# sergivalverde/sub-cortical_segmentation

Hardware: NVIDIA B200
Metric: voxels_per_sec_full_volume_inference (higher is better)
Workload: dtype bf16

## Files before the change

sub-cortical_segmentation_b200/csrc/common.cuh:

```cuda
#pragma once
#include <cuda_bf16.h>
#include <cuda_runtime.h>
#include <nvtx3/nvToolsExt.h>
#include <stdint.h>
#include <stdio.h>
#include <atomic>
#include <string>
#include <utility>
#include <vector>

#include "../../include/subcort_b200.h"

namespace sc {

void set_error(const char* fmt, ...);

#define SC_CUDA(expr)                                                                        \
  do {                                                                                       \
    cudaError_t _e = (expr);                                                                 \
    if (_e != cudaSuccess) {                                                                 \
      sc::set_error("%s:%d: %s -> %s", __FILE__, __LINE__, #expr, cudaGetErrorString(_e));   \
      return SC_ERR_CUDA;                                                                    \
    }                                                                                        \
  } while (0)

#define SC_CHECK(cond, code, ...)   \
  do {                              \
    if (!(cond)) {                  \
      sc::set_error(__VA_ARGS__);   \
      return code;                  \
    }                               \
  } while (0)

#define SC_TRY(expr)           \
  do {                         \
    int _s = (expr);           \
    if (_s != SC_OK) return _s;\
  } while (0)

constexpr int kConvCin[5] = {1, 20, 20, 40, 40};
constexpr int kConvCout[5] = {20, 20, 40, 40, 60};

struct BranchOff {
  int convW[5];
  int bn[5][4];
  int alpha[5];
  int d1W, d1b, d1alpha;
};
struct ParamOff {
  BranchOff br[3];
  int fc1W, fc1b, a1;
  int fc2W, fc2b, a2;
  int outW, outb;
  int total;
};
inline ParamOff make_param_off() {
  ParamOff P;
  int o = 0;
  for (int b = 0; b < 3; ++b) {
    for (int l = 0; l < 5; ++l) {
      P.br[b].convW[l] = o; o += kConvCout[l] * kConvCin[l] * 9;
      for (int k = 0; k < 4; ++k) { P.br[b].bn[l][k] = o; o += kConvCout[l]; }
      P.br[b].alpha[l] = o; o += kConvCout[l];
    }
    P.br[b].d1W = o; o += 540 * 180;
    P.br[b].d1b = o; o += 180;
    P.br[b].d1alpha = o; o += 180;
  }
  P.fc1W = o; o += 540 * 540; P.fc1b = o; o += 540; P.a1 = o; o += 540;
  P.fc2W = o; o += 555 * 270; P.fc2b = o; o += 270; P.a2 = o; o += 270;
  P.outW = o; o += 270 * 15; P.outb = o; o += 15;
  P.total = o;
  return P;
}

constexpr int kFeat = 540;
constexpr int kFeatLd = 576;
constexpr int kH1 = 555;
constexpr int kH1Ld = 576;
constexpr int kH2 = 270;
constexpr int kH2Ld = 272;
constexpr int kH2LdTc = 320;
constexpr int kC5Ld = 64;
constexpr int kD1K = 9 * kC5Ld;

struct GemmW {
  float* w_kn;
  float* w_nk;
  float* bias;
  float* alpha;
  float* scale;
  int K, N, Kpad, Npad;
  int k_used = 0;
};

struct SweepW {
  float* panels;
  float* panels_pair;
  float* scale;
  float* shift;
  float* alpha;
  int bn, ksteps, npanels;
};

struct Conv1Consts { float w[9 * 20]; float scale[20], shift[20], alpha[20]; };

struct BranchW {
  Conv1Consts c1_host;
  float* c1_w;
  float* conv_w[5];
  float* scale[5];
  float* shift[5];
  float* alpha[5];
  SweepW conv_sw[5];
  GemmW d1;
  GemmW d1_dense;
};

struct Workspace {
  void* ptr = nullptr;
  size_t bytes = 0;
};

enum ProfClass {
  PC_GATHER = 0, PC_NONZERO, PC_SCATTER, PC_PATCH_BRANCH, PC_CONV1, PC_CONV2, PC_CONV3, PC_CONV4, PC_CONV5,
  PC_GEMM_D1, PC_GEMM_FC1, PC_GEMM_FC2, PC_ATLAS, PC_OUT, PC_POOL, PC_TRAIN_FWD, PC_TRAIN_BWD, PC_ADAM, PC_COUNT
};
struct ProfEvent { int cls; cudaEvent_t a, b; };

}

struct sc_ctx {
  int device = 0;
  int sm_count = 0;
  bool weights_loaded = false;
  int gemm_backend = 1;
  int64_t chunk_voxels = 1 << 20;
  int64_t launches = 0;
  sc::ParamOff off;
  float* params = nullptr;
  float* grads = nullptr;
  float* adam_m = nullptr;
  float* adam_v = nullptr;
  uint8_t* trainable = nullptr;
  int64_t adam_t = 0;
  float* derived = nullptr;
  size_t derived_floats = 0;
  sc::BranchW br[3];
  sc::GemmW fc1, fc2;
  sc::GemmW outl;
  float* out_w = nullptr;
  float* out_b = nullptr;
  sc::Workspace ws;
  sc::Workspace ws_train;
  sc::Workspace ws_fit;
  struct TrainGraph { int n; long long n_global; int injected; int backend; void* arena; cudaGraphExec_t exec; int launches; };
  std::vector<TrainGraph> train_graphs;
  cudaStream_t train_side[2] = {nullptr, nullptr};
  cudaEvent_t train_ev[8] = {};
  int train_graph_on = 1;
  unsigned* peer_flags = nullptr;
  float* peer_grads[8] = {}; float* peer_params[8] = {}; unsigned* peer_flagp[8] = {};
  int peer_rank = 0, peer_world = 0; unsigned peer_step = 0;
  sc_allreduce_fn ar_hook = nullptr;
  void* ar_user = nullptr;
  void* train_panels = nullptr;
  void* train_dense_w = nullptr;
  struct TrainDenseW { float* wnk; float* wkn; float* bias; };
  TrainDenseW train_dw[6];
  sc::SweepW train_sw[3][5][2];
  float* train_consts = nullptr;
  int64_t* d_count = nullptr;
  int64_t* h_count = nullptr;
  void* tc_state = nullptr;
  int tc_timing_cls = -1;
  unsigned long long* tc_timing_buf = nullptr;
  int train_wgrad_mn = 1;
  int train_fused_stats = 1;
  int tc_skip = 1;
  int tc_compact = 1;
  int32_t* h_slab_cnt = nullptr;
  unsigned char* tile_flags = nullptr;
  size_t tile_flags_cap = 0;
  cudaEvent_t compact_ev = nullptr;
  int gather_ctas_per_sm = 0;
  cudaStream_t copy_stream = nullptr;
  cudaEvent_t copy_ev[2] = {nullptr, nullptr};
  cudaEvent_t atlas_ready = nullptr;
  cudaEvent_t atlas_chunk_ev[64] = {};
  int atlas_chunks = 0, atlas_chunk_nx = 0;
  std::atomic<int>* atlas_recorded = nullptr;
  bool profile = false;
  std::vector<sc::ProfEvent> prof_live;
  std::vector<sc::ProfEvent> prof_free;
  bool derived_dirty = false;
  std::vector<std::pair<const void*, int>> smem_attr;
};

namespace sc {
int ensure_ws(Workspace& ws, size_t bytes);
int ensure_smem_attr(sc_ctx* ctx, const void* kernel, int bytes);

const char* prof_class_name(int cls);
struct ProfScope {
  sc_ctx* ctx; cudaStream_t st; ProfEvent ev; bool on;
  ProfScope(sc_ctx* c, int cls, cudaStream_t s) : ctx(c), st(s), on(c->profile) {
    nvtxRangePushA(prof_class_name(cls));
    if (!on) return;
    if (!ctx->prof_free.empty()) { ev = ctx->prof_free.back(); ctx->prof_free.pop_back(); }
    else { cudaEventCreate(&ev.a); cudaEventCreate(&ev.b); }
    ev.cls = cls;
    cudaEventRecord(ev.a, st);
  }
  ~ProfScope() {
    if (on) {
      cudaEventRecord(ev.b, st);
      ctx->prof_live.push_back(ev);
    }
    nvtxRangePop();
  }
};

struct OutGeo { int x0, y0, z0, by, bz, Y, Z; };

int launch_gather(sc_ctx* ctx, const float* vol, const int32_t* dims, const float* atlas, int bg_fix,
                  const int32_t* xyz, int64_t n, float* ax, float* co, float* sa, float* atlas_out, cudaStream_t st);
int launch_slab_compact(sc_ctx* ctx, const uint8_t* cand, const OutGeo& box, int bx, int nx_per_slab, int32_t* rowmap, int32_t* rowvox,
                        int32_t* cnt, int32_t* scratch, cudaStream_t st);
int launch_center_labels(sc_ctx* ctx, const uint8_t* lab, const int32_t* dims, const int32_t* xyz, int64_t n,
                         uint8_t* y, cudaStream_t st);
int launch_gather_samples(sc_ctx* ctx, const sc_scan* scans, int n_scans, const int32_t* samples, const float* atlas_rows,
                          const uint8_t* labels, const int64_t* idx, int64_t n, float* ax, float* co, float* sa,
                          float* atlas_out, uint8_t* y_out, cudaStream_t st);
int launch_nonzero(sc_ctx* ctx, const void* vol, int elem_bytes, const int32_t* dims, int32_t* xyz,
                   int64_t capacity, int64_t* n_out_host, cudaStream_t st);
int launch_dilate(sc_ctx* ctx, const uint8_t* mask, const int32_t* dims, int iterations, uint8_t* out, cudaStream_t st);
int launch_scatter(sc_ctx* ctx, const int32_t* xyz, int64_t n, const int32_t* label, const float* proba,
                   const int32_t* dims, uint8_t* label_vol, float* proba_vol, cudaStream_t st);

int import_volume(sc_ctx* ctx, const void* src, int elem_bytes, const int32_t* dims, int channels, void* dst, cudaStream_t st);
int upload_volume_box(sc_ctx* ctx, const void* src_host, int elem_bytes, const int32_t* dims, int channels, int fortran_order,
                      const int32_t* box, void* staging_dev, void* dst, cudaStream_t st);
int normalise_volume(sc_ctx* ctx, const void* vol, int dtype, const int32_t* dims, float* out, double* mean_std_host, cudaStream_t st);
int candidate_mask(sc_ctx* ctx, const void* vol, int dtype, const int32_t* dims, uint8_t* mask, cudaStream_t st);
int mask_bbox(sc_ctx* ctx, const uint8_t* mask, const int32_t* dims, int32_t* box_host, int64_t* count_host, cudaStream_t st);

int post_process(sc_ctx* ctx, const uint8_t* seg, const uint8_t* mask, const int32_t* dims, uint8_t* out, cudaStream_t st);

int derive_weights(sc_ctx* ctx, cudaStream_t st);

struct GemmProblem {
  const float* A;
  int64_t lda, a_ys, a_zs;
  int ntaps;
  int64_t tap_off[9];
  int kc;
  float* C;
  int64_t ldc, c_ys, c_zs;
  int M, Y, Z;
  const float* a_base;
  int64_t a_dims[4];
  int64_t a_strides[3];
  int tap_dx[9], tap_dy[9];
  int tap_dz[9] = {0, 0, 0, 0, 0, 0, 0, 0, 0};
  int a_y0, a_z0;
  int prof_cls;
  int k_used;
  int n_store;
  int c_col0;
  int out_split;
  const int32_t* rowmap = nullptr;
  const int32_t* rowvox = nullptr;
  const float* atlas = nullptr;
  OutGeo ageo;
  const struct SoftmaxOut* sm = nullptr;
  int a_swap = 0;
};
int launch_gemm(sc_ctx* ctx, const GemmProblem& p, const GemmW& w, cudaStream_t st);
inline void gemm_problem_rows(GemmProblem& p, const float* A, int64_t lda, int kc, int M) {
  p.c_col0 = 0; p.out_split = 0; p.k_used = 0; p.a_swap = 0;
  p.A = A; p.lda = lda; p.a_ys = p.a_zs = 0; p.ntaps = 1; p.tap_off[0] = 0; p.kc = kc;
  p.M = M; p.Y = p.Z = 1; p.c_ys = p.c_zs = 0;
  p.a_base = A; p.a_dims[0] = kc; p.a_dims[1] = M; p.a_dims[2] = p.a_dims[3] = 1;
  p.a_strides[0] = lda; p.a_strides[1] = p.a_strides[2] = (int64_t)M * lda;
  for (int t = 0; t < 9; ++t) p.tap_dx[t] = p.tap_dy[t] = 0;
  p.a_y0 = p.a_z0 = 0;
}
struct SoftmaxOut { float* proba; int32_t* label32; uint8_t* label8; const uint8_t* mask; OutGeo geo; int use_geo;
                    const int32_t* rowvox; };
int launch_out_softmax(sc_ctx* ctx, const float* h2, int64_t n, float* proba, int32_t* label32, uint8_t* label8,
                       const uint8_t* mask, const OutGeo* geo, cudaStream_t st);

int tc_init(sc_ctx* ctx);
void tc_destroy(sc_ctx* ctx);
int launch_gemm_tc(sc_ctx* ctx, const GemmProblem& p, const GemmW& w, cudaStream_t st);
int launch_split_rows(sc_ctx* ctx, const float* in, int64_t rows, float* out, cudaStream_t st);

struct ViewGeo {
  int64_t ss, rs, cs;
  int s0, ns;
  int r0, c0;
  int br, bc;
  int R, C;
};

int launch_conv1_wide(sc_ctx* ctx, const float* vol, const ViewGeo& g, int ns, const Conv1Consts& cw, float* out, int outR, int outC,
                      cudaStream_t st);
struct SweepStats { double* sums; int H, pitch; };
struct SweepSkip { const uint32_t* occ; int br, bc, ns, C1; uint8_t* flags; };
int launch_view_occupancy(sc_ctx* ctx, const uint8_t* cand, const ViewGeo& g, uint32_t* occ, cudaStream_t st);
int launch_conv_sweep(sc_ctx* ctx, const SweepW& w, int layer, const float* in, int in_fmt, float* out, int out_fmt,
                      int Pw, int R, int rows_out, int dil, int pool, int prof_cls, cudaStream_t st, int in_dx = 0, int in_dy = 0,
                      const SweepSkip* skip = nullptr, const struct SweepStats* stats = nullptr);

int launch_branch_patches(sc_ctx* ctx, int branch, const float* patches, int64_t n, float* c5_out ,
                          cudaStream_t st);
int forward_patches(sc_ctx* ctx, const float* in1, const float* in2, const float* in3, const float* in4, int64_t n,
                    float* proba, int32_t* label, cudaStream_t st);

struct ConvArgs {
  const float* in; int inR, inLd;
  float* out; int outR, outC, outLd;
  const float* w;
  const float* scale; const float* shift; const float* alpha;
  int ns; int round_out;
};
int launch_conv3x3(sc_ctx* ctx, int cin, int cout, const ConvArgs& a, int prof_cls, cudaStream_t st);
int launch_conv1_patches(sc_ctx* ctx, const float* patches, int n, const float* w, const float* scale, const float* shift,
                         const float* alpha, float* out, cudaStream_t st);
size_t branch_patches_tc_bytes(int64_t n);
int branch_patches_tc(sc_ctx* ctx, int branch, const float* patches, int64_t n, float* scratch, float* feats ,
                      cudaStream_t st);
int segment_volume(sc_ctx* ctx, const float* vol, const int32_t* dims, const float* atlas, const int32_t* box,
                   const uint8_t* cand, uint8_t* label_vol, float* proba_vol, cudaStream_t st);

constexpr float kBnEps = 1e-4f;
struct TcBranchBuf {
  float* X[5]; float* A[5]; uint16_t* AT[5]; uint8_t* idx[5]; float* mean[5]; float* istd[5];
  float* frame; float* dA; uint16_t* DT; float* dX0; double* sums;
};
size_t tc_branch_bytes(int n);
int tc_carve_branch(TcBranchBuf& T, char* base, int n);
int tc_branch_forward(sc_ctx* ctx, int b, const TcBranchBuf& T, const float* patches, const float* wf0, int n, const uint8_t* masks,
                      float* F5, cudaStream_t s);
int tc_branch_backward(sc_ctx* ctx, int b, const TcBranchBuf& T, const float* patches, const float* dF5, int dF5_ld, const uint8_t* masks, int n,
                       cudaStream_t s);
constexpr int kTrainZeros = 1024;
struct TcDenseBuf {
  int npad;
  char* zero_begin; size_t zero_bytes;
  float *F5s[3], *F5T[3], *Z1[3], *dZ1s[3], *dZ1T[3], *dF5[3], *gW1[3];
  float *CATs, *CATT, *ZF1, *CAT2s, *CAT2T, *ZF2, *H2s, *H2T, *ZO, *dZOs, *dZOT, *dH2, *dZF2s, *dZF2T, *dCAT2, *dZF1s, *dZF1T, *dCAT;
  float *gWfc1, *gWfc2, *gWout;
};
int tc_train_prepare(sc_ctx* ctx);
int tdense_prepare(sc_ctx* ctx);
size_t tdense_bytes(int n);
void tdense_carve(TcDenseBuf& D, char* base, int n);
int tdense_branch_forward(sc_ctx* ctx, int b, const TcDenseBuf& D, const float* F5, int n, const uint8_t* masks, cudaStream_t s);
int tdense_head(sc_ctx* ctx, const TcDenseBuf& D, const float* in4, const uint8_t* y, int n, int64_t n_global, const uint8_t* masks, float* loss,
                cudaStream_t s);
int tdense_branch_backward(sc_ctx* ctx, int b, const TcDenseBuf& D, int n, const uint8_t* masks, cudaStream_t s);
int launch_conv1_wgrad(sc_ctx* ctx, const float* patches, const float* dx_planar, int n, int zc, float* gW, cudaStream_t st);

int fused_export(sc_ctx* ctx, unsigned char* handles);
int fused_attach(sc_ctx* ctx, int rank, int world, const unsigned char* all);
void fused_detach(sc_ctx* ctx);
int fused_allreduce_adam(sc_ctx* ctx, float lr, float b1, float b2, float eps, cudaStream_t st);

int train_forward_backward(sc_ctx* ctx, const float* in1, const float* in2, const float* in3, const float* in4,
                           const uint8_t* y, int64_t n, int64_t n_global, uint64_t seed, const uint8_t* masks,
                           float* loss, cudaStream_t st);
int adam_step(sc_ctx* ctx, float lr, float b1, float b2, float eps, float gscale, float sscale, cudaStream_t st);
int eval_batch(sc_ctx* ctx, const float* in1, const float* in2, const float* in3, const float* in4, const uint8_t* y,
               int64_t n, float* out2, cudaStream_t st);

__device__ __forceinline__ float prelu(float x, float a) { return x > 0.f ? x : a * x; }
__device__ __forceinline__ void store_split4(float* row, int n, float v0, float v1, float v2, float v3) {
  __nv_bfloat16* r = reinterpret_cast<__nv_bfloat16*>(row) + (n >> 6) * 128 + (n & 63);
  const __nv_bfloat16 h0 = __float2bfloat16_rn(v0), h1 = __float2bfloat16_rn(v1), h2 = __float2bfloat16_rn(v2), h3 = __float2bfloat16_rn(v3);
  const __nv_bfloat16 l0 = __float2bfloat16_rn(v0 - __bfloat162float(h0)), l1 = __float2bfloat16_rn(v1 - __bfloat162float(h1));
  const __nv_bfloat16 l2 = __float2bfloat16_rn(v2 - __bfloat162float(h2)), l3 = __float2bfloat16_rn(v3 - __bfloat162float(h3));
  uint2 hp, lp;
  hp.x = (uint32_t)__bfloat16_as_ushort(h0) | ((uint32_t)__bfloat16_as_ushort(h1) << 16);
  hp.y = (uint32_t)__bfloat16_as_ushort(h2) | ((uint32_t)__bfloat16_as_ushort(h3) << 16);
  lp.x = (uint32_t)__bfloat16_as_ushort(l0) | ((uint32_t)__bfloat16_as_ushort(l1) << 16);
  lp.y = (uint32_t)__bfloat16_as_ushort(l2) | ((uint32_t)__bfloat16_as_ushort(l3) << 16);
  *reinterpret_cast<uint2*>(r) = hp;
  *reinterpret_cast<uint2*>(r + 64) = lp;
}
__device__ __forceinline__ void store_split4_b32(void* px, int n, float v0, float v1, float v2, float v3) {
  __nv_bfloat16* r = reinterpret_cast<__nv_bfloat16*>(px) + n;
  const __nv_bfloat16 h0 = __float2bfloat16_rn(v0), h1 = __float2bfloat16_rn(v1), h2 = __float2bfloat16_rn(v2), h3 = __float2bfloat16_rn(v3);
  const __nv_bfloat16 l0 = __float2bfloat16_rn(v0 - __bfloat162float(h0)), l1 = __float2bfloat16_rn(v1 - __bfloat162float(h1));
  const __nv_bfloat16 l2 = __float2bfloat16_rn(v2 - __bfloat162float(h2)), l3 = __float2bfloat16_rn(v3 - __bfloat162float(h3));
  uint2 hp, lp;
  hp.x = (uint32_t)__bfloat16_as_ushort(h0) | ((uint32_t)__bfloat16_as_ushort(h1) << 16);
  hp.y = (uint32_t)__bfloat16_as_ushort(h2) | ((uint32_t)__bfloat16_as_ushort(h3) << 16);
  lp.x = (uint32_t)__bfloat16_as_ushort(l0) | ((uint32_t)__bfloat16_as_ushort(l1) << 16);
  lp.y = (uint32_t)__bfloat16_as_ushort(l2) | ((uint32_t)__bfloat16_as_ushort(l3) << 16);
  *reinterpret_cast<uint2*>(r) = hp;
  *reinterpret_cast<uint2*>(r + 32) = lp;
}
__device__ __forceinline__ void store_row1(float* row, int n, int split, float v) {
  if (!split) { row[n] = v; return; }
  __nv_bfloat16* r = reinterpret_cast<__nv_bfloat16*>(row) + (n >> 6) * 128 + (n & 63);
  const __nv_bfloat16 h = __float2bfloat16_rn(v);
  r[0] = h;
  r[64] = __float2bfloat16_rn(v - __bfloat162float(h));
}
__device__ __forceinline__ void store_row4(float* row, int n, int split, float v0, float v1, float v2, float v3) {
  if (split) store_split4(row, n, v0, v1, v2, v3);
  else *reinterpret_cast<float4*>(row + n) = make_float4(v0, v1, v2, v3);
}
}
```

sub-cortical_segmentation_b200/csrc/dense.cu:

```cuda
#include <thread>

#include "common.cuh"

namespace sc {


__host__ __device__ inline int round8(int v) { return (v + 7) & ~7; }

__global__ void __launch_bounds__(256) dense_conv1_kernel(const float* __restrict__ vol, ViewGeo g, int sbeg, int ns,
                                                          const float* __restrict__ w, const float* __restrict__ scale,
                                                          const float* __restrict__ shift, const float* __restrict__ alpha,
                                                          float* __restrict__ out, int outR, int ld) {
  __shared__ float sw[9 * 20], ssc[20], ssh[20], sal[20];
  for (int i = threadIdx.x; i < 180; i += 256) sw[i] = w[i];
  if (threadIdx.x < 20) { ssc[threadIdx.x] = scale[threadIdx.x]; ssh[threadIdx.x] = shift[threadIdx.x]; sal[threadIdx.x] = alpha[threadIdx.x]; }
  __syncthreads();
  const int quads = ld >> 2;
  const int64_t total = (int64_t)ns * outR * quads;
  for (int64_t e = (int64_t)blockIdx.x * 256 + threadIdx.x; e < total; e += (int64_t)gridDim.x * 256) {
    const int q = (int)(e % quads);
    const int i = (int)((e / quads) % outR);
    const int s = (int)(e / ((int64_t)quads * outR));
    const int j0 = q * 4;
    float x[3][6];
    const float* base = vol + (int64_t)(g.s0 + sbeg + s) * g.ss;
#pragma unroll
    for (int ky = 0; ky < 3; ++ky) {
      const int rr = g.r0 + i + ky - 16;
      const bool rin = rr >= 0 && rr < g.R;
#pragma unroll
      for (int t = 0; t < 6; ++t) {
        const int cc = g.c0 + j0 + t - 16;
        x[ky][t] = (rin && cc >= 0 && cc < g.C) ? __ldg(base + (int64_t)rr * g.rs + (int64_t)cc * g.cs) : 0.f;
      }
    }
    float* o = out + (((int64_t)s * 20) * outR + i) * ld + j0;
    const int64_t plane = (int64_t)outR * ld;
#pragma unroll 4
    for (int co = 0; co < 20; ++co) {
      float a0 = 0.f, a1 = 0.f, a2 = 0.f, a3 = 0.f;
#pragma unroll
      for (int ky = 0; ky < 3; ++ky)
#pragma unroll
        for (int kx = 0; kx < 3; ++kx) {
          const float wv = sw[(ky * 3 + kx) * 20 + co];
          a0 = fmaf(x[ky][kx + 0], wv, a0); a1 = fmaf(x[ky][kx + 1], wv, a1);
          a2 = fmaf(x[ky][kx + 2], wv, a2); a3 = fmaf(x[ky][kx + 3], wv, a3);
        }
      const float sc_ = ssc[co], sh = ssh[co], al = sal[co];
      float4 v;
      v.x = prelu(fmaf(a0, sc_, sh), al); v.y = prelu(fmaf(a1, sc_, sh), al);
      v.z = prelu(fmaf(a2, sc_, sh), al); v.w = prelu(fmaf(a3, sc_, sh), al);
      *reinterpret_cast<float4*>(o + co * plane) = v;
    }
  }
}

template <int CIN, int COUT, int DIL, int POOLD, bool NHWC_OUT>
struct ConvCfg {
  static constexpr int TH = 16, TW = 32, CHUNK = 10;
  static constexpr int CO_T = COUT / 5;
  static constexpr int IH = TH + 2 * DIL;
  static constexpr int NV = (8 + 2 * DIL + 3) / 4;
  static constexpr int IW = 24 + NV * 4;
  static constexpr int IWP = (IW % 8 == 4) ? IW : IW + 4;
  static constexpr int IN_FLOATS = CHUNK * IH * IWP;
  static constexpr int W_FLOATS = CHUNK * 9 * COUT;
  static constexpr size_t SMEM = (size_t)(IN_FLOATS + W_FLOATS) * sizeof(float);
};

template <int CIN, int COUT, int DIL, int POOLD, bool NHWC_OUT>
__global__ void __launch_bounds__(320) dense_conv_kernel(const ConvArgs a) {
  using Cfg = ConvCfg<CIN, COUT, DIL, POOLD, NHWC_OUT>;
  extern __shared__ __align__(16) float smem[];
  float* s_in = smem;
  float* s_w = smem + Cfg::IN_FLOATS;
  const int tid = threadIdx.x;
  const int cg = tid >> 6, pg = tid & 63, prow = pg >> 2, pseg = pg & 3;
  const int tr0 = blockIdx.y * Cfg::TH, tc0 = blockIdx.x * Cfg::TW;
  const int s = blockIdx.z;
  const float* in_s = a.in + (int64_t)s * CIN * a.inR * a.inLd;

  float acc[8][Cfg::CO_T];
#pragma unroll
  for (int p = 0; p < 8; ++p)
#pragma unroll
    for (int c = 0; c < Cfg::CO_T; ++c) acc[p][c] = 0.f;

  for (int ci0 = 0; ci0 < CIN; ci0 += Cfg::CHUNK) {
    __syncthreads();
    for (int e = tid; e < Cfg::CHUNK * Cfg::IH * Cfg::IW; e += 320) {
      const int col = e % Cfg::IW;
      const int row = (e / Cfg::IW) % Cfg::IH;
      const int ci = e / (Cfg::IW * Cfg::IH);
      const int gr = tr0 + row, gc = tc0 + col;
      float v = 0.f;
      if (gr + POOLD < a.inR && gc + POOLD < a.inLd) {
        const float* p = in_s + ((int64_t)(ci0 + ci) * a.inR + gr) * a.inLd + gc;
        v = __ldg(p);
        if (POOLD > 0) {
          v = fmaxf(v, __ldg(p + POOLD));
          v = fmaxf(v, fmaxf(__ldg(p + (int64_t)POOLD * a.inLd), __ldg(p + (int64_t)POOLD * a.inLd + POOLD)));
        }
      }
      s_in[(ci * Cfg::IH + row) * Cfg::IWP + col] = v;
    }
    for (int e = tid; e < Cfg::W_FLOATS / 4; e += 320)
      reinterpret_cast<float4*>(s_w)[e] = __ldg(reinterpret_cast<const float4*>(a.w + (int64_t)ci0 * 9 * COUT) + e);
    __syncthreads();

#pragma unroll 1
    for (int ci = 0; ci < Cfg::CHUNK; ++ci) {
#pragma unroll
      for (int ky = 0; ky < 3; ++ky) {
        float x[Cfg::NV * 4];
        const float4* src = reinterpret_cast<const float4*>(s_in + (ci * Cfg::IH + prow + ky * DIL) * Cfg::IWP + pseg * 8);
#pragma unroll
        for (int v = 0; v < Cfg::NV; ++v) {
          const float4 t = src[v];
          x[v * 4 + 0] = t.x; x[v * 4 + 1] = t.y; x[v * 4 + 2] = t.z; x[v * 4 + 3] = t.w;
        }
#pragma unroll
        for (int kx = 0; kx < 3; ++kx) {
          float wv[Cfg::CO_T];
          const float4* wsrc = reinterpret_cast<const float4*>(s_w + (ci * 9 + ky * 3 + kx) * COUT + cg * Cfg::CO_T);
#pragma unroll
          for (int v = 0; v < Cfg::CO_T / 4; ++v) {
            const float4 t = wsrc[v];
            wv[v * 4 + 0] = t.x; wv[v * 4 + 1] = t.y; wv[v * 4 + 2] = t.z; wv[v * 4 + 3] = t.w;
          }
#pragma unroll
          for (int p = 0; p < 8; ++p)
#pragma unroll
            for (int c = 0; c < Cfg::CO_T; ++c) acc[p][c] = fmaf(x[kx * DIL + p], wv[c], acc[p][c]);
        }
      }
    }
  }

  const int orow = tr0 + prow, ocol = tc0 + pseg * 8;
  if (orow >= a.outR) return;
  if (!NHWC_OUT) {
    if (ocol >= a.outLd) return;
#pragma unroll
    for (int c = 0; c < Cfg::CO_T; ++c) {
      const int co = cg * Cfg::CO_T + c;
      const float sc_ = __ldg(a.scale + co), sh = __ldg(a.shift + co), al = __ldg(a.alpha + co);
      float r[8];
#pragma unroll
      for (int p = 0; p < 8; ++p) r[p] = prelu(fmaf(acc[p][c], sc_, sh), al);
      float* o = a.out + (((int64_t)s * COUT + co) * a.outR + orow) * a.outLd + ocol;
      *reinterpret_cast<float4*>(o) = make_float4(r[0], r[1], r[2], r[3]);
      *reinterpret_cast<float4*>(o + 4) = make_float4(r[4], r[5], r[6], r[7]);
    }
  } else {
    float sc_[Cfg::CO_T], sh[Cfg::CO_T], al[Cfg::CO_T];
#pragma unroll
    for (int c = 0; c < Cfg::CO_T; ++c) {
      const int co = cg * Cfg::CO_T + c;
      sc_[c] = __ldg(a.scale + co); sh[c] = __ldg(a.shift + co); al[c] = __ldg(a.alpha + co);
    }
#pragma unroll
    for (int p = 0; p < 8; ++p) {
      if (ocol + p >= a.outC) break;
      float* o = a.out + (((int64_t)s * a.outR + orow) * a.outC + ocol + p) * kC5Ld;
#pragma unroll
      for (int v = 0; v < Cfg::CO_T / 4; ++v) {
        float r[4];
#pragma unroll
        for (int k = 0; k < 4; ++k) r[k] = prelu(fmaf(acc[p][v * 4 + k], sc_[v * 4 + k], sh[v * 4 + k]), al[v * 4 + k]);
        store_row4(o, cg * Cfg::CO_T + v * 4, a.round_out, r[0], r[1], r[2], r[3]);
      }
      if (cg == 4 && COUT < kC5Ld) store_row4(o, COUT, a.round_out, 0.f, 0.f, 0.f, 0.f);
    }
  }
}

template <int CIN, int COUT, int DIL, int POOLD, bool NHWC_OUT>
static int launch_dense_conv(sc_ctx* ctx, const ConvArgs& a, int prof_cls, cudaStream_t st) {
  using Cfg = ConvCfg<CIN, COUT, DIL, POOLD, NHWC_OUT>;
  auto kern = dense_conv_kernel<CIN, COUT, DIL, POOLD, NHWC_OUT>;
  SC_TRY(ensure_smem_attr(ctx, reinterpret_cast<const void*>(kern), (int)Cfg::SMEM));
  const int width = NHWC_OUT ? a.outC : a.outLd;
  dim3 grid((width + Cfg::TW - 1) / Cfg::TW, (a.outR + Cfg::TH - 1) / Cfg::TH, a.ns);
  ProfScope prof(ctx, prof_cls, st);
  kern<<<grid, 320, Cfg::SMEM, st>>>(a);
  ctx->launches++;
  SC_CUDA(cudaGetLastError());
  return SC_OK;
}

size_t branch_patches_tc_bytes(int64_t n) {
  return (size_t)n * ((960 + 240) * 32 + (240 + 56 + 56) * 64) * sizeof(float) + 5 * 256;
}

int branch_patches_tc(sc_ctx* ctx, int b, const float* patches, int64_t n, float* scratch, float* feats, cudaStream_t st) {
  const BranchW& W = ctx->br[b];
  auto carve = [&](float*& cur, size_t floats) { float* p = cur; cur += (floats + 63) & ~(size_t)63; return p; };
  float* cur = scratch;
  float* c1 = carve(cur, (size_t)n * 960 * 32);
  float* p1 = carve(cur, (size_t)n * 240 * 32);
  float* c3 = carve(cur, (size_t)n * 240 * 64);
  float* p2 = carve(cur, (size_t)n * 56 * 64);
  float* c5 = carve(cur, (size_t)n * 56 * 64);
  SC_CHECK(n * 960 < (1ll << 31), SC_ERR_ARG, "patchwise chunk too large");
  {
    ViewGeo g = {1024, 32, 1, 0, (int)n, 16, 16, 30, 30, 32, 32};
    SC_TRY(launch_conv1_wide(ctx, patches, g, (int)n, W.c1_host, c1, 30, 32, st));
  }
  SC_TRY(launch_conv_sweep(ctx, W.conv_sw[1], 1, c1, 1, p1, 1, (int)(n * 32), 30, 28, 1, 2, PC_CONV2, st));
  SC_TRY(launch_conv_sweep(ctx, W.conv_sw[2], 2, p1, 1, c3, 0, (int)(n * 16), 15, 12, 1, 0, PC_CONV3, st));
  SC_TRY(launch_conv_sweep(ctx, W.conv_sw[3], 3, c3, 0, p2, 0, (int)(n * 16), 15, 10, 1, 2, PC_CONV4, st));
  SC_TRY(launch_conv_sweep(ctx, W.conv_sw[4], 4, p2, 0, c5, 0, (int)(n * 8), 7, 3, 1, 0, PC_CONV5, st));
  GemmProblem p;
  p.A = c5; p.lda = 8 * kC5Ld; p.a_ys = 0; p.a_zs = 0;
  p.ntaps = 9; p.kc = kC5Ld; p.k_used = 0;
  for (int t = 0; t < 9; ++t) {
    p.tap_dx[t] = 0; p.tap_dy[t] = t % 3; p.tap_dz[t] = t / 3;
    p.tap_off[t] = ((int64_t)(t / 3) * n * 8 + (t % 3)) * kC5Ld;
  }
  p.a_base = c5; p.a_dims[0] = kC5Ld; p.a_dims[1] = n; p.a_dims[2] = 8; p.a_dims[3] = 7;
  p.a_strides[0] = 8 * kC5Ld; p.a_strides[1] = kC5Ld; p.a_strides[2] = (int64_t)n * 8 * kC5Ld;
  p.a_y0 = p.a_z0 = 0;
  p.C = feats; p.ldc = kFeatLd; p.c_ys = p.c_zs = 0; p.M = (int)n; p.Y = p.Z = 1;
  p.n_store = 192; p.c_col0 = b * 192; p.out_split = 1; p.prof_cls = PC_GEMM_D1;
  SC_TRY(launch_gemm_tc(ctx, p, W.d1_dense, st));
  SC_CUDA(cudaGetLastError());
  return SC_OK;
}

int launch_conv3x3(sc_ctx* ctx, int cin, int cout, const ConvArgs& a, int prof_cls, cudaStream_t st) {
  if (cin == 20 && cout == 20) return launch_dense_conv<20, 20, 1, 0, false>(ctx, a, prof_cls, st);
  if (cin == 20 && cout == 40) return launch_dense_conv<20, 40, 1, 0, false>(ctx, a, prof_cls, st);
  if (cin == 40 && cout == 40) return launch_dense_conv<40, 40, 1, 0, false>(ctx, a, prof_cls, st);
  if (cin == 40 && cout == 60) return launch_dense_conv<40, 60, 1, 0, false>(ctx, a, prof_cls, st);
  if (cin == 60 && cout == 40) return launch_dense_conv<60, 40, 1, 0, false>(ctx, a, prof_cls, st);
  if (cin == 40 && cout == 20) return launch_dense_conv<40, 20, 1, 0, false>(ctx, a, prof_cls, st);
  set_error("launch_conv3x3: unsupported channel pair %d -> %d", cin, cout);
  return SC_ERR_ARG;
}

int launch_conv1_patches(sc_ctx* ctx, const float* patches, int n, const float* w, const float* scale, const float* shift,
                         const float* alpha, float* out, cudaStream_t st) {
  ViewGeo g = {1024, 32, 1, 0, n, 16, 16, 30, 30, 32, 32};
  const int64_t work = (int64_t)n * 30 * 8;
  const int64_t blocks = (work + 255) / 256;
  const unsigned grid = (unsigned)(blocks < (int64_t)ctx->sm_count * 32 ? blocks : (int64_t)ctx->sm_count * 32);
  ProfScope prof(ctx, PC_TRAIN_FWD, st);
  dense_conv1_kernel<<<grid, 256, 0, st>>>(patches, g, 0, n, w, scale, shift, alpha, out, 30, 32);
  ctx->launches++;
  SC_CUDA(cudaGetLastError());
  return SC_OK;
}

__global__ void dense_atlas_kernel(const float* __restrict__ atlas, OutGeo g, int ix0, int64_t rows, float* __restrict__ h1,
                                   int split) {
  const int64_t m = (int64_t)blockIdx.x * blockDim.x + threadIdx.x;
  if (m >= rows) return;
  const int64_t plane = (int64_t)g.by * g.bz;
  const int ix = (int)(m / plane);
  const int rem = (int)(m - (int64_t)ix * plane);
  const int iy = rem / g.bz, iz = rem - iy * g.bz;
  const int64_t v = ((int64_t)(g.x0 + ix0 + ix) * g.Y + (g.y0 + iy)) * g.Z + (g.z0 + iz);
  float a[16];
#pragma unroll
  for (int c = 0; c < 15; ++c) a[c] = __ldg(atlas + v * 15 + c);
  float s = __fadd_rn(__fadd_rn(__fadd_rn(a[0], a[1]), __fadd_rn(a[2], a[3])),
                      __fadd_rn(__fadd_rn(a[4], a[5]), __fadd_rn(a[6], a[7])));
#pragma unroll
  for (int k = 8; k < 15; ++k) s = __fadd_rn(s, a[k]);
  if (s == 0.f) a[14] = 1.f;
  a[15] = 0.f;
  float* hr = h1 + m * kH1Ld;
#pragma unroll
  for (int q = 0; q < 9; ++q) {
    if (q < 4) store_row4(hr, 540 + 4 * q, split, a[4 * q], a[4 * q + 1], a[4 * q + 2], a[4 * q + 3]);
    else store_row4(hr, 540 + 4 * q, split, 0.f, 0.f, 0.f, 0.f);
  }
}

static size_t align256(size_t v) { return (v + 255) & ~(size_t)255; }

int segment_volume(sc_ctx* ctx, const float* vol, const int32_t* dims, const float* atlas, const int32_t* box,
                   const uint8_t* cand, uint8_t* label_vol, float* proba_vol, cudaStream_t st) {
  const int X = dims[0], Y = dims[1], Z = dims[2];
  int b[6] = {0, X, 0, Y, 0, Z};
  if (box) for (int i = 0; i < 6; ++i) b[i] = box[i];
  SC_CHECK(b[0] >= 0 && b[1] <= X && b[2] >= 0 && b[3] <= Y && b[4] >= 0 && b[5] <= Z, SC_ERR_ARG, "sc_segment_volume: box outside the volume");
  const int bx = b[1] - b[0], by = b[3] - b[2], bz = b[5] - b[4];
  if (bx <= 0 || by <= 0 || bz <= 0) return SC_OK;
  const int64_t YZ = (int64_t)Y * Z;
  const bool tc = ctx->gemm_backend == 1;

  ViewGeo vg[3];
  vg[0] = {1, YZ, Z, b[4], bz, b[0], b[2], bx, by, X, Y};
  vg[1] = {Z, YZ, 1, b[2], by, b[0], b[4], bx, bz, X, Z};
  vg[2] = {YZ, Z, 1, b[0], bx, b[2], b[4], by, bz, Y, Z};

  size_t a5_off[3], a5_bytes = 0;
  for (int v = 0; v < 3; ++v) {
    a5_off[v] = a5_bytes;
    a5_bytes += tc ? align256((size_t)vg[v].ns * (vg[v].br + 29) * (vg[v].bc + 29) * kC5Ld * sizeof(float))
                   : align256((size_t)vg[v].ns * (vg[v].br + 8) * (vg[v].bc + 8) * kC5Ld * sizeof(float));
  }
  size_t per_slice_max = 0, view_max = 0;
  for (int v = 0; v < 3; ++v) {
    const size_t br = vg[v].br, bc = vg[v].bc;
    size_t f;
    if (tc) {
      f = (size_t)vg[v].ns * (br + 29) * (bc + 29) * (2 * 32 + 2 * 64) + 4 * 64;
      view_max = f > view_max ? f : view_max;
      continue;
    }
    f = 20 * (br + 29) * round8(bc + 29) + 20 * (br + 27) * round8(bc + 27) + 40 * (br + 22) * round8(bc + 22) +
        40 * (br + 18) * round8(bc + 18);
    per_slice_max = f > per_slice_max ? f : per_slice_max;
  }
  const size_t scratch_budget = (size_t)1536 << 20;
  int group = tc ? 1 : (int)(scratch_budget / (per_slice_max * sizeof(float) + 1024));
  if (group < 1) group = 1;
  if (group > 64) group = 64;
  const size_t scratch_bytes = tc ? align256(view_max * sizeof(float) + 4096) : align256((per_slice_max * sizeof(float) + 1024) * group);
  const int64_t plane = (int64_t)by * bz;
  int slab = (int)(ctx->chunk_voxels / plane);
  if (slab < 1) slab = 1;
  if (slab > bx) slab = bx;
  const size_t rows_max = (size_t)slab * plane;
  const size_t feat_bytes = align256(rows_max * kFeatLd * sizeof(float));
  const size_t h1_bytes = align256(rows_max * kH1Ld * sizeof(float));
  const int h2ld = tc ? kH2LdTc : kH2Ld;
  const size_t h2_bytes = align256(rows_max * h2ld * sizeof(float));
  const int nslabs = (bx + slab - 1) / slab;
  bool compact = tc && cand != nullptr && ctx->tc_compact && nslabs <= 4096;
  const size_t nbox = (size_t)bx * plane;
  const size_t cmp_blocks = (size_t)nslabs * ((rows_max + 2047) / 2048);
  const size_t cmp_bytes = compact ? align256(nbox * 4) * 2 + align256(cmp_blocks * 8 + 16) + align256((size_t)nslabs * 4) : 0;
  size_t occ_off[3], skip_bytes = 0;
  for (int v = 0; v < 3; ++v) { occ_off[v] = skip_bytes; skip_bytes += compact ? align256((size_t)vg[v].br * vg[v].ns * 4) : 0; }
  const size_t flags_off = skip_bytes;
  if (compact) skip_bytes += align256((size_t)1 << 20);
  const size_t total = a5_bytes + scratch_bytes + feat_bytes + h1_bytes + h2_bytes + cmp_bytes + skip_bytes;
  SC_TRY(ensure_ws(ctx->ws, total));
  char* wsb = reinterpret_cast<char*>(ctx->ws.ptr);
  float* a5[3] = {reinterpret_cast<float*>(wsb + a5_off[0]), reinterpret_cast<float*>(wsb + a5_off[1]),
                  reinterpret_cast<float*>(wsb + a5_off[2])};
  char* scratch = wsb + a5_bytes;
  float* feats = reinterpret_cast<float*>(scratch + scratch_bytes);
  float* h1 = reinterpret_cast<float*>(reinterpret_cast<char*>(feats) + feat_bytes);
  float* h2 = reinterpret_cast<float*>(reinterpret_cast<char*>(h1) + h1_bytes);
  int32_t* rowmap = reinterpret_cast<int32_t*>(reinterpret_cast<char*>(h2) + h2_bytes);
  int32_t* rowvox = reinterpret_cast<int32_t*>(reinterpret_cast<char*>(rowmap) + align256(nbox * 4));
  int32_t* cmp_scratch = reinterpret_cast<int32_t*>(reinterpret_cast<char*>(rowvox) + align256(nbox * 4));
  int32_t* d_slab_cnt = reinterpret_cast<int32_t*>(reinterpret_cast<char*>(cmp_scratch) + align256(cmp_blocks * 8 + 16));
  char* skip_base = wsb + (total - skip_bytes);
  if (compact) {
    if (!ctx->h_slab_cnt) {
      SC_CUDA(cudaMallocHost(&ctx->h_slab_cnt, 4096 * sizeof(int32_t)));
      SC_CUDA(cudaEventCreateWithFlags(&ctx->compact_ev, cudaEventDisableTiming));
    }
    OutGeo boxg = {b[0], b[2], b[4], by, bz, Y, Z};
    SC_TRY(launch_slab_compact(ctx, cand, boxg, bx, slab, rowmap, rowvox, d_slab_cnt, cmp_scratch, st));
    SC_CUDA(cudaMemcpyAsync(ctx->h_slab_cnt, d_slab_cnt, (size_t)nslabs * sizeof(int32_t), cudaMemcpyDeviceToHost, st));
    SC_CUDA(cudaEventRecord(ctx->compact_ev, st));
    SC_CUDA(cudaEventSynchronize(ctx->compact_ev));
    int64_t ncand = 0;
    for (int i = 0; i < nslabs; ++i) ncand += ctx->h_slab_cnt[i];
    if (ncand * 10 >= (int64_t)nbox * 9) compact = false;
  }
  SweepSkip skips[3];
  const bool skip_on = compact && ctx->tc_skip;
  if (skip_on) {
    for (int v = 0; v < 3; ++v) {
      uint32_t* occ = reinterpret_cast<uint32_t*>(skip_base + occ_off[v]);
      SC_TRY(launch_view_occupancy(ctx, cand, vg[v], occ, st));
      skips[v] = {occ, vg[v].br, vg[v].bc, vg[v].ns, vg[v].bc + 29, reinterpret_cast<uint8_t*>(skip_base + flags_off)};
    }
  }

  for (int v = 0; v < 3; ++v) {
    const ViewGeo& g = vg[v];
    const BranchW& W = ctx->br[v];
    const int r1 = g.br + 29, l1 = round8(g.bc + 29);
    const int r2 = g.br + 27, l2 = round8(g.bc + 27);
    const int r3 = g.br + 22, l3 = round8(g.bc + 22);
    const int r4 = g.br + 18, l4 = round8(g.bc + 18);
    const int r5 = g.br + 8, c5 = g.bc + 8;
    if (tc) {
      const int R1 = g.br + 29, C1 = g.bc + 29;
      const int64_t Pw64 = (int64_t)g.ns * C1;
      const int64_t npos = Pw64 * R1;
      SC_CHECK(npos < (1ll << 31), SC_ERR_ARG, "sc_segment_volume: view too large");
      const int Pw = (int)Pw64;
      auto carve = [&](float*& cur, int px_floats) { float* p = cur; cur += align256((size_t)npos * px_floats * 4) / 4; return p; };
      float* cur = reinterpret_cast<float*>(scratch);
      float* m1 = carve(cur, 32); float* mp1 = carve(cur, 32);
      float* m3 = carve(cur, 64); float* mp2 = carve(cur, 64);
      SC_TRY(launch_conv1_wide(ctx, vol, g, g.ns, W.c1_host, m1, R1, C1, st));
      const SweepSkip* sk = skip_on ? &skips[v] : nullptr;
      SC_TRY(launch_conv_sweep(ctx, W.conv_sw[1], 1, m1, 1, mp1, 1, Pw, R1, g.br + 26, 1, 1, PC_CONV2, st, 0, 0, sk));
      SC_TRY(launch_conv_sweep(ctx, W.conv_sw[2], 2, mp1, 1, m3, 0, Pw, R1, g.br + 22, 2, 0, PC_CONV3, st, 0, 0, sk));
      SC_TRY(launch_conv_sweep(ctx, W.conv_sw[3], 3, m3, 0, mp2, 0, Pw, R1, g.br + 16, 2, 1, PC_CONV4, st, 0, 0, sk));
      SC_TRY(launch_conv_sweep(ctx, W.conv_sw[4], 4, mp2, 0, a5[v], 0, Pw, R1, g.br + 8, 4, 0, PC_CONV5, st, 0, 0, sk));
      SC_CUDA(cudaGetLastError());
    }
    for (int sb = 0; sb < g.ns && !tc; sb += group) {
      const int ns = g.ns - sb < group ? g.ns - sb : group;
      float* c1 = reinterpret_cast<float*>(scratch);
      float* c2 = c1 + align256((size_t)ns * 20 * r1 * l1 * 4) / 4;
      float* c3 = c2 + align256((size_t)ns * 20 * r2 * l2 * 4) / 4;
      float* c4 = c3 + align256((size_t)ns * 40 * r3 * l3 * 4) / 4;
      {
        const int64_t work = (int64_t)ns * r1 * (l1 / 4);
        const int64_t blocks = (work + 255) / 256;
        const unsigned grid = (unsigned)(blocks < (int64_t)ctx->sm_count * 32 ? blocks : (int64_t)ctx->sm_count * 32);
        ProfScope prof(ctx, PC_CONV1, st);
        dense_conv1_kernel<<<grid, 256, 0, st>>>(vol, g, sb, ns, W.c1_w, W.scale[0], W.shift[0], W.alpha[0], c1, r1, l1);
        ctx->launches++;
        SC_CUDA(cudaGetLastError());
      }
      ConvArgs a;
      a.ns = ns; a.round_out = 0;
      a.in = c1; a.inR = r1; a.inLd = l1; a.out = c2; a.outR = r2; a.outC = g.bc + 27; a.outLd = l2;
      a.w = W.conv_w[1]; a.scale = W.scale[1]; a.shift = W.shift[1]; a.alpha = W.alpha[1];
      SC_TRY((launch_dense_conv<20, 20, 1, 0, false>(ctx, a, PC_CONV2, st)));
      a.in = c2; a.inR = r2; a.inLd = l2; a.out = c3; a.outR = r3; a.outC = g.bc + 22; a.outLd = l3;
      a.w = W.conv_w[2]; a.scale = W.scale[2]; a.shift = W.shift[2]; a.alpha = W.alpha[2];
      SC_TRY((launch_dense_conv<20, 40, 2, 1, false>(ctx, a, PC_CONV3, st)));
      a.in = c3; a.inR = r3; a.inLd = l3; a.out = c4; a.outR = r4; a.outC = g.bc + 18; a.outLd = l4;
      a.w = W.conv_w[3]; a.scale = W.scale[3]; a.shift = W.shift[3]; a.alpha = W.alpha[3];
      SC_TRY((launch_dense_conv<40, 40, 2, 0, false>(ctx, a, PC_CONV4, st)));
      a.in = c4; a.inR = r4; a.inLd = l4; a.out = a5[v] + (size_t)sb * r5 * c5 * kC5Ld; a.outR = r5; a.outC = c5; a.outLd = c5;
      a.w = W.conv_w[4]; a.scale = W.scale[4]; a.shift = W.shift[4]; a.alpha = W.alpha[4];
      a.round_out = tc ? 1 : 0;
      SC_TRY((launch_dense_conv<40, 60, 4, 2, true>(ctx, a, PC_CONV5, st)));
    }
  }

  int atlas_waited = 0;
  OutGeo og = {b[0], b[2], b[4], by, bz, Y, Z};
  if (tc) SC_CUDA(cudaMemsetAsync(h2, 0, h2_bytes, st));
  for (int ix0 = 0; ix0 < bx; ix0 += slab) {
    const int nx = bx - ix0 < slab ? bx - ix0 : slab;
    const int64_t rows = (int64_t)nx * plane;
    if (ctx->atlas_chunks > 0) {
      int need = (b[0] + ix0 + nx + ctx->atlas_chunk_nx - 1) / ctx->atlas_chunk_nx;
      if (need > ctx->atlas_chunks) need = ctx->atlas_chunks;
      if (need > atlas_waited) {
        if (ctx->atlas_recorded)
          while (ctx->atlas_recorded->load(std::memory_order_acquire) < need) std::this_thread::yield();
        SC_CUDA(cudaStreamWaitEvent(st, ctx->atlas_chunk_ev[need - 1], 0));
        atlas_waited = need;
      }
    }
    const int64_t slab_base = (int64_t)ix0 * plane;
    const int64_t rows_fc = compact ? ctx->h_slab_cnt[ix0 / slab] : rows;
    if (rows_fc == 0) continue;
    for (int v = 0; v < 3; ++v) {
      const ViewGeo& g = vg[v];
      const int64_t c5 = tc ? g.bc + 29 : g.bc + 8, r5 = tc ? g.br + 29 : g.br + 8;
      GemmProblem p;
      p.lda = kC5Ld; p.a_ys = c5 * kC5Ld; p.a_zs = r5 * c5 * kC5Ld;
      p.ntaps = 9; p.kc = kC5Ld;
      for (int t = 0; t < 9; ++t) {
        p.tap_off[t] = ((int64_t)(t / 3) * 4 * c5 + (t % 3) * 4) * kC5Ld;
        p.tap_dx[t] = (t % 3) * 4; p.tap_dy[t] = (t / 3) * 4;
      }
      p.a_base = a5[v]; p.a_dims[0] = kC5Ld; p.a_dims[1] = c5; p.a_dims[2] = r5; p.a_dims[3] = g.ns;
      p.a_strides[0] = kC5Ld; p.a_strides[1] = c5 * kC5Ld; p.a_strides[2] = r5 * c5 * kC5Ld;
      p.a_swap = 0;
      if (tc) {
        p.a_dims[2] = g.ns; p.a_dims[3] = r5;
        p.a_strides[1] = c5 * kC5Ld; p.a_strides[2] = (int64_t)g.ns * c5 * kC5Ld;
        p.a_swap = 1;
      }
      p.a_y0 = v == 2 ? 0 : ix0; p.a_z0 = v == 2 ? ix0 : 0;
      p.ldc = 0; p.out_split = tc ? 1 : 0; p.c_col0 = v * 192; p.prof_cls = PC_GEMM_D1; p.k_used = 0;
      p.n_store = 192;
      if (v == 0) {
        p.A = a5[0] + (int64_t)ix0 * p.a_ys; p.M = by; p.Y = nx; p.Z = bz;
        p.ldc = (int64_t)bz * kFeatLd; p.c_ys = plane * kFeatLd; p.c_zs = kFeatLd;
      } else if (v == 1) {
        p.A = a5[1] + (int64_t)ix0 * p.a_ys; p.M = bz; p.Y = nx; p.Z = by;
        p.ldc = kFeatLd; p.c_ys = plane * kFeatLd; p.c_zs = (int64_t)bz * kFeatLd;
      } else {
        p.A = a5[2] + (int64_t)ix0 * p.a_zs; p.M = bz; p.Y = by; p.Z = nx;
        p.ldc = kFeatLd; p.c_ys = (int64_t)bz * kFeatLd; p.c_zs = plane * kFeatLd;
      }
      p.C = feats;
      if (compact) p.rowmap = rowmap + slab_base;
      SC_TRY(tc ? launch_gemm_tc(ctx, p, ctx->br[v].d1_dense, st) : launch_gemm(ctx, p, ctx->br[v].d1_dense, st));
    }
    GemmProblem p;
    SC_CHECK(rows < (1ll << 31), SC_ERR_ARG, "sc_segment_volume: chunk too large");
    gemm_problem_rows(p, feats, kFeatLd, kFeatLd, (int)rows_fc);
    p.C = h1; p.ldc = kH1Ld; p.n_store = 540; p.out_split = tc ? 1 : 0;
    p.prof_cls = PC_GEMM_FC1;
    const bool atlas_fused = tc;
    if (ctx->atlas_ready && ctx->atlas_chunks == 0) {
      SC_CUDA(cudaStreamWaitEvent(st, ctx->atlas_ready, 0));
      ctx->atlas_ready = nullptr;
    }
    if (atlas_fused) { p.atlas = atlas; p.ageo = og; p.ageo.x0 = b[0] + ix0; if (compact) p.rowvox = rowvox + slab_base; }
    SC_TRY(tc ? launch_gemm_tc(ctx, p, ctx->fc1, st) : launch_gemm(ctx, p, ctx->fc1, st));
    p.atlas = nullptr; p.rowvox = nullptr;
    if (!atlas_fused) {
      ProfScope prof(ctx, PC_ATLAS, st);
      dense_atlas_kernel<<<(unsigned)((rows + 255) / 256), 256, 0, st>>>(atlas, og, ix0, rows, h1, tc ? 1 : 0);
      ctx->launches++;
    }
    SC_CUDA(cudaGetLastError());
    gemm_problem_rows(p, h1, kH1Ld, kH1Ld, (int)rows_fc);
    p.C = h2; p.ldc = h2ld; p.n_store = kH2Ld; p.out_split = tc ? 1 : 0;
    p.prof_cls = PC_GEMM_FC2;
    SC_TRY(tc ? launch_gemm_tc(ctx, p, ctx->fc2, st) : launch_gemm(ctx, p, ctx->fc2, st));
    OutGeo og2 = og;
    og2.x0 = b[0] + ix0;
    if (tc) {
      SoftmaxOut smo = {proba_vol, nullptr, label_vol, cand, og2, 1, compact ? rowvox + slab_base : nullptr};
      gemm_problem_rows(p, h2, h2ld, h2ld, (int)rows_fc);
      p.C = nullptr; p.ldc = 0; p.n_store = 16; p.out_split = 0; p.sm = &smo;
      p.prof_cls = PC_OUT;
      SC_TRY(launch_gemm_tc(ctx, p, ctx->outl, st));
    } else {
      SC_TRY(launch_out_softmax(ctx, h2, rows, proba_vol, nullptr, label_vol, cand, &og2, st));
    }
  }
  if (ctx->atlas_ready && ctx->atlas_chunks == 0) {
    SC_CUDA(cudaStreamWaitEvent(st, ctx->atlas_ready, 0));
    ctx->atlas_ready = nullptr;
  }
  return SC_OK;
}

}
```

sub-cortical_segmentation_b200/csrc/gemm_simt.cu:

```cuda
#include "common.cuh"

namespace sc {

constexpr int BM = 128, BN = 64, BK = 16;
constexpr int AS_LD = BM + 4;

struct GemmArgs {
  GemmProblem p;
  const float* W;
  const float* bias;
  const float* alpha;
  int Npad;
  int mt, nt;
};

__global__ void __launch_bounds__(256) gemm_simt_kernel(const GemmArgs a) {
  __shared__ __align__(16) float As[BK][AS_LD];
  __shared__ __align__(16) float Bs[BK][BN];
  const GemmProblem& p = a.p;
  int64_t bid = blockIdx.x;
  const int n_tile = (int)(bid % a.nt); bid /= a.nt;
  const int m_tile = (int)(bid % a.mt); bid /= a.mt;
  const int y = (int)(bid % p.Y);
  const int z = (int)(bid / p.Y);
  const int m0 = m_tile * BM, n0 = n_tile * BN;
  const float* Abase = p.A + (int64_t)z * p.a_zs + (int64_t)y * p.a_ys;
  const int tid = threadIdx.x, tm = tid & 15, tn = tid >> 4;

  float acc[8][4];
#pragma unroll
  for (int i = 0; i < 8; ++i)
#pragma unroll
    for (int j = 0; j < 4; ++j) acc[i][j] = 0.f;

  for (int tap = 0; tap < p.ntaps; ++tap) {
    const float* At = Abase + p.tap_off[tap];
    const float* Wt = a.W + (int64_t)tap * p.kc * a.Npad;
    for (int k0 = 0; k0 < p.kc; k0 += BK) {
#pragma unroll
      for (int r = 0; r < 2; ++r) {
        const int idx = tid + r * 256, row = idx >> 2, kq = idx & 3;
        float4 v = make_float4(0.f, 0.f, 0.f, 0.f);
        if (m0 + row < p.M) v = __ldg(reinterpret_cast<const float4*>(At + (int64_t)(m0 + row) * p.lda + k0 + kq * 4));
        As[kq * 4 + 0][row] = v.x; As[kq * 4 + 1][row] = v.y; As[kq * 4 + 2][row] = v.z; As[kq * 4 + 3][row] = v.w;
      }
      {
        const int kr = tid >> 4, nq = tid & 15;
        float4 v = make_float4(0.f, 0.f, 0.f, 0.f);
        if (n0 + nq * 4 < a.Npad) v = __ldg(reinterpret_cast<const float4*>(Wt + (int64_t)(k0 + kr) * a.Npad + n0 + nq * 4));
        *reinterpret_cast<float4*>(&Bs[kr][nq * 4]) = v;
      }
      __syncthreads();
#pragma unroll
      for (int k = 0; k < BK; ++k) {
        const float4 a0 = *reinterpret_cast<const float4*>(&As[k][tm * 8]);
        const float4 a1 = *reinterpret_cast<const float4*>(&As[k][tm * 8 + 4]);
        const float4 b = *reinterpret_cast<const float4*>(&Bs[k][tn * 4]);
        const float av[8] = {a0.x, a0.y, a0.z, a0.w, a1.x, a1.y, a1.z, a1.w};
        const float bv[4] = {b.x, b.y, b.z, b.w};
#pragma unroll
        for (int i = 0; i < 8; ++i)
#pragma unroll
          for (int j = 0; j < 4; ++j) acc[i][j] = fmaf(av[i], bv[j], acc[i][j]);
      }
      __syncthreads();
    }
  }
  const int n = n0 + tn * 4;
  if (n >= p.n_store) return;
  const float4 bias = __ldg(reinterpret_cast<const float4*>(a.bias + n));
  const float4 al = __ldg(reinterpret_cast<const float4*>(a.alpha + n));
  float* Cbase = p.C + (int64_t)z * p.c_zs + (int64_t)y * p.c_ys;
#pragma unroll
  for (int i = 0; i < 8; ++i) {
    const int m = m0 + tm * 8 + i;
    if (m >= p.M) break;
    float4 v;
    v.x = prelu(acc[i][0] + bias.x, al.x);
    v.y = prelu(acc[i][1] + bias.y, al.y);
    v.z = prelu(acc[i][2] + bias.z, al.z);
    v.w = prelu(acc[i][3] + bias.w, al.w);
    *reinterpret_cast<float4*>(Cbase + (int64_t)m * p.ldc + p.c_col0 + n) = v;
  }
}

int launch_gemm(sc_ctx* ctx, const GemmProblem& p, const GemmW& w, cudaStream_t st) {
  if (p.M <= 0 || p.Y <= 0 || p.Z <= 0) return SC_OK;
  SC_CHECK(p.kc % BK == 0 && p.n_store % 4 == 0 && p.n_store <= w.Npad, SC_ERR_ARG, "gemm: bad geometry kc=%d n_store=%d", p.kc, p.n_store);
  SC_CHECK(p.ntaps * p.kc == w.Kpad, SC_ERR_ARG, "gemm: K mismatch %d*%d vs %d", p.ntaps, p.kc, w.Kpad);
  SC_CHECK(!p.out_split && p.c_col0 % 4 == 0, SC_ERR_ARG, "gemm: the SIMT back-end writes plain fp32 rows only");
  GemmArgs a;
  a.p = p; a.W = w.w_kn; a.bias = w.bias; a.alpha = w.alpha; a.Npad = w.Npad;
  a.mt = (p.M + BM - 1) / BM;
  a.nt = (p.n_store + BN - 1) / BN;
  const int64_t blocks = (int64_t)a.mt * a.nt * p.Y * p.Z;
  SC_CHECK(blocks < (1ll << 31), SC_ERR_ARG, "gemm: grid too large");
  ProfScope prof(ctx, p.prof_cls, st);
  gemm_simt_kernel<<<(unsigned)blocks, 256, 0, st>>>(a);
  ctx->launches++;
  SC_CUDA(cudaGetLastError());
  return SC_OK;
}

__global__ void __launch_bounds__(128) out_softmax_kernel(const float* __restrict__ h2, int64_t n,
                                                          const float* __restrict__ W, const float* __restrict__ b,
                                                          float* __restrict__ proba, int32_t* __restrict__ label,
                                                          uint8_t* __restrict__ label8, const uint8_t* __restrict__ mask,
                                                          const OutGeo geo, const int use_geo) {
  __shared__ __align__(16) float sW[270 * 16];
  for (int i = threadIdx.x; i < 270 * 16; i += 128) sW[i] = W[i];
  __syncthreads();
  const int64_t v = (int64_t)blockIdx.x * 128 + threadIdx.x;
  if (v >= n) return;
  int64_t o = v;
  if (use_geo) {
    const int64_t plane = (int64_t)geo.by * geo.bz;
    const int ix = (int)(v / plane);
    const int rem = (int)(v - (int64_t)ix * plane);
    const int iy = rem / geo.bz, iz = rem - iy * geo.bz;
    o = ((int64_t)(geo.x0 + ix) * geo.Y + (geo.y0 + iy)) * geo.Z + (geo.z0 + iz);
    if (mask && mask[o] == 0) return;
  }
  const float4* row = reinterpret_cast<const float4*>(h2 + v * kH2Ld);
  float z[15];
#pragma unroll
  for (int c = 0; c < 15; ++c) z[c] = __ldg(b + c);
#pragma unroll 2
  for (int k4 = 0; k4 < 68; ++k4) {
    const float4 xv = __ldg(row + k4);
    const float x[4] = {xv.x, xv.y, xv.z, xv.w};
#pragma unroll
    for (int j = 0; j < 4; ++j) {
      const int k = k4 * 4 + j;
      if (k < 270) {
        const float4* w4 = reinterpret_cast<const float4*>(sW + k * 16);
        const float4 w0 = w4[0], w1 = w4[1], w2 = w4[2], w3 = w4[3];
        z[0] = fmaf(x[j], w0.x, z[0]); z[1] = fmaf(x[j], w0.y, z[1]); z[2] = fmaf(x[j], w0.z, z[2]); z[3] = fmaf(x[j], w0.w, z[3]);
        z[4] = fmaf(x[j], w1.x, z[4]); z[5] = fmaf(x[j], w1.y, z[5]); z[6] = fmaf(x[j], w1.z, z[6]); z[7] = fmaf(x[j], w1.w, z[7]);
        z[8] = fmaf(x[j], w2.x, z[8]); z[9] = fmaf(x[j], w2.y, z[9]); z[10] = fmaf(x[j], w2.z, z[10]); z[11] = fmaf(x[j], w2.w, z[11]);
        z[12] = fmaf(x[j], w3.x, z[12]); z[13] = fmaf(x[j], w3.y, z[13]); z[14] = fmaf(x[j], w3.z, z[14]);
      }
    }
  }
  float mx = z[0];
#pragma unroll
  for (int c = 1; c < 15; ++c) mx = fmaxf(mx, z[c]);
  float sum = 0.f;
#pragma unroll
  for (int c = 0; c < 15; ++c) { z[c] = expf(z[c] - mx); sum += z[c]; }
  const float inv = 1.f / sum;
  int best = 0;
  float bp = z[0] * inv;
#pragma unroll
  for (int c = 0; c < 15; ++c) {
    z[c] *= inv;
    if (z[c] > bp) { bp = z[c]; best = c; }
  }
  if (proba) {
#pragma unroll
    for (int c = 0; c < 15; ++c) proba[o * 15 + c] = z[c];
  }
  if (label) label[o] = best;
  if (label8) label8[o] = (uint8_t)best;
}

int launch_out_softmax(sc_ctx* ctx, const float* h2, int64_t n, float* proba, int32_t* label, uint8_t* label8,
                       const uint8_t* mask, const OutGeo* geo, cudaStream_t st) {
  if (n == 0) return SC_OK;
  const int64_t blocks = (n + 127) / 128;
  SC_CHECK(blocks < (1ll << 31), SC_ERR_ARG, "out_softmax: too many rows");
  const unsigned grid = (unsigned)blocks;
  OutGeo g = geo ? *geo : OutGeo{0, 0, 0, 1, 1, 1, 1};
  ProfScope prof(ctx, PC_OUT, st);
  out_softmax_kernel<<<grid, 128, 0, st>>>(h2, n, ctx->out_w, ctx->out_b, proba, label, label8, mask, g, geo ? 1 : 0);
  ctx->launches++;
  SC_CUDA(cudaGetLastError());
  return SC_OK;
}

}
```

sub-cortical_segmentation_b200/csrc/gemm_tc.cu:

```cuda
#include "tc_common.cuh"

namespace sc {

__device__ __forceinline__ void tmem_ld16(uint32_t (&r)[16], uint32_t taddr) {
  asm volatile(
      "tcgen05.ld.sync.aligned.32x32b.x16.b32 {%0, %1, %2, %3, %4, %5, %6, %7, %8, %9, %10, %11, %12, %13, %14, %15}, [%16];"
      : "=r"(r[0]), "=r"(r[1]), "=r"(r[2]), "=r"(r[3]), "=r"(r[4]), "=r"(r[5]), "=r"(r[6]), "=r"(r[7]), "=r"(r[8]),
        "=r"(r[9]), "=r"(r[10]), "=r"(r[11]), "=r"(r[12]), "=r"(r[13]), "=r"(r[14]), "=r"(r[15])
      : "r"(taddr));
}

constexpr int TC_BM = 128;
constexpr int TC_BK = 64;
constexpr int TC_A_HALF = TC_BM * 128;

struct TcArgs {
  int kpt;
  int nkb;
  int stages;
  int bn;
  int nt, mt;
  int Y;
  int M;
  int n_store, npad, c_col0;
  int a_y0, a_z0;
  int a_swap;
  int tap_dx[9], tap_dy[9], tap_dz[9];
  float* C;
  long long ldc, c_ys, c_zs;
  const float* bias;
  const float* alpha;
  const float* scale;
  int out_split;
  long long num_tiles;
  int epi_warps;
  int last_ksteps;
  unsigned long long* dbg;
  const int* rowmap;
  const int* rowvox;
  long long crow_ld;
  int n_mma;
  const unsigned char* tile_on;
  const float* atlas;
  OutGeo ageo;
  int sm_on;
  SoftmaxOut sm;
};


__global__ void __launch_bounds__(576, 1)
gemm_tc_persistent_kernel(const __grid_constant__ CUtensorMap mapA, const __grid_constant__ CUtensorMap mapB, const TcArgs a) {
  extern __shared__ uint8_t smem_raw[];
  uint8_t* smem = smem_raw + ((1024u - (smem_u32(smem_raw) & 1023u)) & 1023u);
  const int b_half = a.bn * 128;
  const int w_block = 2 * b_half;
  const int stage_bytes = 2 * TC_A_HALF + w_block;
  uint8_t* sStage = smem;
  uint64_t* bars = reinterpret_cast<uint64_t*>(sStage + a.stages * stage_bytes);
  uint64_t* full = bars;
  uint64_t* empty = bars + a.stages;
  uint64_t* tfull = bars + 2 * a.stages;
  uint64_t* tempty = tfull + 2;
  uint32_t* tmem_slot = reinterpret_cast<uint32_t*>(tempty + 2);
  float* s_const = reinterpret_cast<float*>(tmem_slot + 4);
  uint8_t* s_stage = reinterpret_cast<uint8_t*>(s_const + 2 * 3 * a.bn);

  const int warp = threadIdx.x >> 5, lane = threadIdx.x & 31;

  if (threadIdx.x == 0) {
    for (int s = 0; s < a.stages; ++s) { mbar_init(&full[s], 1); mbar_init(&empty[s], 1); }
    for (int b = 0; b < 2; ++b) { mbar_init(&tfull[b], 1); mbar_init(&tempty[b], (blockDim.x >> 5) - 2); }
    asm volatile("fence.mbarrier_init.release.cluster;" ::: "memory");
  }
  if (warp == 1) {
    asm volatile("tcgen05.alloc.cta_group::1.sync.aligned.shared::cta.b32 [%0], %1;" ::"r"(smem_u32(tmem_slot)), "r"(512) : "memory");
    asm volatile("tcgen05.relinquish_alloc_permit.cta_group::1.sync.aligned;" ::: "memory");
  }
  asm volatile("tcgen05.fence::before_thread_sync;" ::: "memory");
  __syncthreads();
  asm volatile("tcgen05.fence::after_thread_sync;" ::: "memory");
  const uint32_t tmem_base = *tmem_slot;

  if (warp == 0) {
    if (lane == 0) {
      asm volatile("prefetch.tensormap [%0];" ::"l"(reinterpret_cast<uint64_t>(&mapA)) : "memory");
      asm volatile("prefetch.tensormap [%0];" ::"l"(reinterpret_cast<uint64_t>(&mapB)) : "memory");
      uint32_t it = 0;
      long long dbg_acc[1] = {0};
      const long long tstart = a.dbg ? clock64() : 0;
      for (long long t = blockIdx.x; t < a.num_tiles; t += gridDim.x) {
        long long r = t;
        const int n_tile = (int)(r % a.nt); r /= a.nt;
        const int m_tile = (int)(r % a.mt); r /= a.mt;
        const int y = (int)(r % a.Y);
        const int z = (int)(r / a.Y);
        const int m0 = m_tile * TC_BM, n0 = n_tile * a.bn;
        for (int kb = 0; kb < a.nkb; ++kb, ++it) {
          const int s = it % a.stages;
          const uint32_t use = it / a.stages;
          if (use > 0) {
            const long long c0 = a.dbg ? clock64() : 0;
            mbar_wait(&empty[s], (use - 1) & 1);
            if (a.dbg) dbg_acc[0] += clock64() - c0;
          }
          mbar_expect_tx(&full[s], (uint32_t)stage_bytes);
          uint8_t* sp = sStage + s * stage_bytes;
          const int tap = kb / a.kpt, ka = (kb - tap * a.kpt) * 2 * TC_BK;
          const int px = m0 + a.tap_dx[tap], ln = y + a.a_y0 + a.tap_dy[tap], pl = z + a.a_z0 + a.tap_dz[tap];
          tma_load_4d(&mapA, &full[s], sp, ka, px, a.a_swap ? pl : ln, a.a_swap ? ln : pl);
          tma_load_4d(&mapA, &full[s], sp + TC_A_HALF, ka + TC_BK, px, a.a_swap ? pl : ln, a.a_swap ? ln : pl);
          tma_load_2d(&mapB, &full[s], sp + 2 * TC_A_HALF, kb * 2 * TC_BK, n0);
          tma_load_2d(&mapB, &full[s], sp + 2 * TC_A_HALF + b_half, kb * 2 * TC_BK + TC_BK, n0);
        }
      }
      if (a.dbg) { a.dbg[blockIdx.x * 8 + 0] = (unsigned long long)dbg_acc[0]; a.dbg[blockIdx.x * 8 + 1] = (unsigned long long)(clock64() - tstart); }
    }
    __syncwarp();
  } else if (warp == 1) {
    const uint32_t leader = elect_one();
    const uint32_t idesc = (1u << 4) | (1u << 7) | (1u << 10) | ((uint32_t)(a.bn >> 3) << 17) | ((uint32_t)(TC_BM >> 4) << 24);
    const uint32_t sStage_u = smem_u32(sStage);
    uint32_t it = 0, ti = 0;
    long long w_full = 0, w_tempty = 0;
    const long long tstart = a.dbg ? clock64() : 0;
    for (long long t = blockIdx.x; t < a.num_tiles; t += gridDim.x, ++ti) {
      const uint32_t b = ti & 1, buse = ti >> 1;
      long long c0 = a.dbg ? clock64() : 0;
      mbar_wait(&tempty[b], (buse & 1) ^ 1);
      if (a.dbg) w_tempty += clock64() - c0;
      asm volatile("tcgen05.fence::after_thread_sync;" ::: "memory");
      const uint32_t acc = tmem_base + b * 256;
      for (int kb = 0; kb < a.nkb; ++kb, ++it) {
        const int s = it % a.stages;
        c0 = a.dbg ? clock64() : 0;
        mbar_wait(&full[s], (it / a.stages) & 1);
        if (a.dbg) w_full += clock64() - c0;
        asm volatile("tcgen05.fence::after_thread_sync;" ::: "memory");
        const uint32_t sp = sStage_u + s * stage_bytes;
        const uint64_t ah = umma_desc(sp), al = umma_desc(sp + TC_A_HALF);
        const uint64_t wh = umma_desc(sp + 2 * TC_A_HALF), wl = umma_desc(sp + 2 * TC_A_HALF + b_half);
#pragma unroll
        for (int j = 0; j < 4; ++j) {
          const uint64_t o = (uint64_t)(j * 2);
          umma_bf16_elect(acc, al + o, wh + o, idesc, (kb | j) != 0, leader);
          umma_bf16_elect(acc, ah + o, wl + o, idesc, 1, leader);
          umma_bf16_elect(acc, ah + o, wh + o, idesc, 1, leader);
        }
        if (leader) umma_commit(&empty[s]);
        __syncwarp();
      }
      if (leader) umma_commit(&tfull[b]);
      __syncwarp();
    }
    if (a.dbg && leader) {
      a.dbg[blockIdx.x * 8 + 2] = (unsigned long long)w_full; a.dbg[blockIdx.x * 8 + 3] = (unsigned long long)w_tempty;
      a.dbg[blockIdx.x * 8 + 4] = (unsigned long long)(clock64() - tstart);
    }
  } else {
    const int q = warp & 3;
    const int nepi = (blockDim.x >> 5) - 2, G = nepi >> 2, grp = (warp - 2) >> 2;
    const int epi_threads = nepi * 32;
    uint32_t ti = 0;
    long long w_tfull = 0;
    const long long tstart = a.dbg ? clock64() : 0;
    for (long long t = blockIdx.x; t < a.num_tiles; t += gridDim.x, ++ti) {
      long long r = t;
      const int n_tile = (int)(r % a.nt); r /= a.nt;
      const int m_tile = (int)(r % a.mt); r /= a.mt;
      const int y = (int)(r % a.Y);
      const int z = (int)(r / a.Y);
      const int m0 = m_tile * TC_BM, n0 = n_tile * a.bn;
      const uint32_t b = ti & 1, buse = ti >> 1;
      float* cb = s_const + b * 3 * a.bn;
      if (ti < 2 || a.nt > 1) {
        for (int i = threadIdx.x - 64; i < a.bn; i += epi_threads) {
          const int nn = n0 + i;
          const bool ok = nn < a.npad;
          cb[i] = ok ? __ldg(a.bias + nn) : 0.f;
          cb[a.bn + i] = ok ? __ldg(a.alpha + nn) : 1.f;
          cb[2 * a.bn + i] = (a.scale && ok) ? __ldg(a.scale + nn) : 1.f;
        }
        asm volatile("bar.sync 1, %0;" ::"r"(epi_threads) : "memory");
      }
      const long long c0w = a.dbg ? clock64() : 0;
      mbar_wait(&tfull[b], buse & 1);
      if (a.dbg) w_tfull += clock64() - c0w;
      asm volatile("tcgen05.fence::after_thread_sync;" ::: "memory");
      float* ctile = a.C + (long long)z * a.c_zs + (long long)y * a.c_ys;
      const int mw = m0 + q * 32;
      uint8_t* stg = s_stage + (warp - 2) * 2560;
      uint8_t* mine = stg + lane * 80;
      if (a.sm_on) {
        if (grp == 0) {
          uint32_t rr[16];
          const uint32_t taddr = tmem_base + b * 256 + ((uint32_t)(q * 32) << 16);
          asm volatile(
              "tcgen05.ld.sync.aligned.32x32b.x16.b32 {%0, %1, %2, %3, %4, %5, %6, %7, %8, %9, %10, %11, %12, %13, %14, %15}, [%16];"
              : "=r"(rr[0]), "=r"(rr[1]), "=r"(rr[2]), "=r"(rr[3]), "=r"(rr[4]), "=r"(rr[5]), "=r"(rr[6]), "=r"(rr[7]), "=r"(rr[8]),
                "=r"(rr[9]), "=r"(rr[10]), "=r"(rr[11]), "=r"(rr[12]), "=r"(rr[13]), "=r"(rr[14]), "=r"(rr[15])
              : "r"(taddr));
          asm volatile("tcgen05.wait::ld.sync.aligned;" ::: "memory");
          long long m = (long long)mw + lane;
          bool ok = m < a.M;
          if (ok && a.sm.rowvox) m = __ldg(a.sm.rowvox + m);
          long long o = m;
          if (ok && a.sm.use_geo) {
            const long long plane = (long long)a.sm.geo.by * a.sm.geo.bz;
            const int ix = (int)(m / plane);
            const int rem = (int)(m - (long long)ix * plane);
            const int iy = rem / a.sm.geo.bz, iz = rem - iy * a.sm.geo.bz;
            o = ((long long)(a.sm.geo.x0 + ix) * a.sm.geo.Y + (a.sm.geo.y0 + iy)) * a.sm.geo.Z + (a.sm.geo.z0 + iz);
            if (a.sm.mask && a.sm.mask[o] == 0) ok = false;
          }
          if (ok) {
            float zz[15];
#pragma unroll
            for (int c = 0; c < 15; ++c) zz[c] = __uint_as_float(rr[c]) + cb[c];
            float mx = zz[0];
#pragma unroll
            for (int c = 1; c < 15; ++c) mx = fmaxf(mx, zz[c]);
            float sum = 0.f;
#pragma unroll
            for (int c = 0; c < 15; ++c) { zz[c] = expf(zz[c] - mx); sum += zz[c]; }
            const float inv = 1.f / sum;
            int best = 0;
            float bp = zz[0] * inv;
#pragma unroll
            for (int c = 0; c < 15; ++c) {
              zz[c] *= inv;
              if (zz[c] > bp) { bp = zz[c]; best = c; }
            }
            if (a.sm.proba) {
#pragma unroll
              for (int c = 0; c < 15; ++c) a.sm.proba[o * 15 + c] = zz[c];
            }
            if (a.sm.label32) a.sm.label32[o] = best;
            if (a.sm.label8) a.sm.label8[o] = (uint8_t)best;
          }
        }
        asm volatile("tcgen05.fence::before_thread_sync;" ::: "memory");
        __syncwarp();
        if (lane == 0) mbar_arrive(&tempty[b]);
        continue;
      }
      for (int c0 = grp * 16; c0 < a.bn; c0 += 16 * G) {
        uint32_t rr[16];
        const uint32_t taddr = tmem_base + b * 256 + ((uint32_t)(q * 32) << 16) + (uint32_t)c0;
        asm volatile(
            "tcgen05.ld.sync.aligned.32x32b.x16.b32 {%0, %1, %2, %3, %4, %5, %6, %7, %8, %9, %10, %11, %12, %13, %14, %15}, [%16];"
            : "=r"(rr[0]), "=r"(rr[1]), "=r"(rr[2]), "=r"(rr[3]), "=r"(rr[4]), "=r"(rr[5]), "=r"(rr[6]), "=r"(rr[7]), "=r"(rr[8]),
              "=r"(rr[9]), "=r"(rr[10]), "=r"(rr[11]), "=r"(rr[12]), "=r"(rr[13]), "=r"(rr[14]), "=r"(rr[15])
            : "r"(taddr));
        asm volatile("tcgen05.wait::ld.sync.aligned;" ::: "memory");
        if (n0 + c0 >= a.n_store) continue;
        float v[16];
#pragma unroll
        for (int k4 = 0; k4 < 4; ++k4) {
          const float4 bi = *reinterpret_cast<const float4*>(cb + c0 + 4 * k4);
          const float4 al = *reinterpret_cast<const float4*>(cb + a.bn + c0 + 4 * k4);
          const float4 sc_ = *reinterpret_cast<const float4*>(cb + 2 * a.bn + c0 + 4 * k4);
          v[4 * k4 + 0] = prelu(fmaf(__uint_as_float(rr[4 * k4 + 0]), sc_.x, bi.x), al.x);
          v[4 * k4 + 1] = prelu(fmaf(__uint_as_float(rr[4 * k4 + 1]), sc_.y, bi.y), al.y);
          v[4 * k4 + 2] = prelu(fmaf(__uint_as_float(rr[4 * k4 + 2]), sc_.z, bi.z), al.z);
          v[4 * k4 + 3] = prelu(fmaf(__uint_as_float(rr[4 * k4 + 3]), sc_.w, bi.w), al.w);
        }
        const int ncol = a.c_col0 + n0 + c0;
        if (a.out_split) {
          uint32_t hi[8], lo[8];
#pragma unroll
          for (int k = 0; k < 8; ++k) split2(v[2 * k], v[2 * k + 1], hi[k], lo[k]);
          *reinterpret_cast<uint4*>(mine) = make_uint4(hi[0], hi[1], hi[2], hi[3]);
          *reinterpret_cast<uint4*>(mine + 16) = make_uint4(hi[4], hi[5], hi[6], hi[7]);
          *reinterpret_cast<uint4*>(mine + 32) = make_uint4(lo[0], lo[1], lo[2], lo[3]);
          *reinterpret_cast<uint4*>(mine + 48) = make_uint4(lo[4], lo[5], lo[6], lo[7]);
          __syncwarp();
          const int boff = (ncol >> 6) * 128 + (ncol & 63);
#pragma unroll
          for (int i = 0; i < 4; ++i) {
            const int half = i >> 1, row = (i & 1) * 16 + (lane >> 1), part = lane & 1;
            const uint4 d = *reinterpret_cast<const uint4*>(stg + row * 80 + half * 32 + part * 16);
            if (mw + row < a.M) {
              __nv_bfloat16* dst = reinterpret_cast<__nv_bfloat16*>(ctile + (long long)(mw + row) * a.ldc) + boff + half * 64 + part * 8;
              *reinterpret_cast<uint4*>(dst) = d;
            }
          }
        } else {
#pragma unroll
          for (int k = 0; k < 4; ++k)
            *reinterpret_cast<float4*>(mine + 16 * k) = make_float4(v[4 * k], v[4 * k + 1], v[4 * k + 2], v[4 * k + 3]);
          __syncwarp();
#pragma unroll
          for (int i = 0; i < 4; ++i) {
            const int row = i * 8 + (lane >> 2), part = lane & 3;
            const float4 d = *reinterpret_cast<const float4*>(stg + row * 80 + part * 16);
            if (mw + row < a.M) *reinterpret_cast<float4*>(ctile + (long long)(mw + row) * a.ldc + ncol + part * 4) = d;
          }
        }
        __syncwarp();
      }
      asm volatile("tcgen05.fence::before_thread_sync;" ::: "memory");
      __syncwarp();
      if (lane == 0) mbar_arrive(&tempty[b]);
    }
    if (a.dbg && threadIdx.x == 64) {
      a.dbg[blockIdx.x * 8 + 5] = (unsigned long long)w_tfull; a.dbg[blockIdx.x * 8 + 6] = (unsigned long long)(clock64() - tstart);
      a.dbg[blockIdx.x * 8 + 7] = ti;
    }
  }
  asm volatile("tcgen05.fence::before_thread_sync;" ::: "memory");
  __syncthreads();
  if (warp == 1) {
    asm volatile("tcgen05.fence::after_thread_sync;" ::: "memory");
    asm volatile("tcgen05.dealloc.cta_group::1.sync.aligned.b32 %0, %1;" ::"r"(tmem_base), "r"(512) : "memory");
  }
}

__global__ void __cluster_dims__(2, 1, 1) __launch_bounds__(576, 1)
gemm_tc_pair_kernel(const __grid_constant__ CUtensorMap mapA, const __grid_constant__ CUtensorMap mapB, const TcArgs a) {
  extern __shared__ uint8_t smem_raw[];
  uint8_t* smem = smem_raw + ((1024u - (smem_u32(smem_raw) & 1023u)) & 1023u);
  const int hb = a.bn >> 1;
  const int b_half = hb * 128;
  const int stage_bytes = 2 * TC_A_HALF + 2 * b_half;
  uint8_t* sStage = smem;
  uint64_t* bars = reinterpret_cast<uint64_t*>(sStage + a.stages * stage_bytes);
  uint64_t* full = bars;
  uint64_t* empty = bars + a.stages;
  uint64_t* tfull = bars + 2 * a.stages;
  uint64_t* tempty = tfull + 2;
  uint32_t* tmem_slot = reinterpret_cast<uint32_t*>(tempty + 2);
  float* s_const = reinterpret_cast<float*>(smem + (((size_t)a.stages * stage_bytes + (2 * a.stages + 4) * 8 + 16 + 15) & ~(size_t)15));
  uint8_t* s_stage = reinterpret_cast<uint8_t*>(s_const + (a.nt > 2 ? a.nt : 2) * 3 * a.bn);

  const int warp = threadIdx.x >> 5, lane = threadIdx.x & 31;
  const uint32_t rank = cluster_ctarank();
  const int nepi = (blockDim.x >> 5) - 2;
  const long long pair = (long long)(blockIdx.x >> 1), npairs = (long long)(gridDim.x >> 1);

  if (threadIdx.x == 0) {
    for (int s = 0; s < a.stages; ++s) { mbar_init(&full[s], 1); mbar_init(&empty[s], 1); }
    for (int b = 0; b < 2; ++b) { mbar_init(&tfull[b], 1); mbar_init(&tempty[b], 2 * nepi); }
    asm volatile("fence.mbarrier_init.release.cluster;" ::: "memory");
  }
  if (warp == 1) {
    asm volatile("tcgen05.alloc.cta_group::2.sync.aligned.shared::cta.b32 [%0], %1;" ::"r"(smem_u32(tmem_slot)), "r"(512) : "memory");
    asm volatile("tcgen05.relinquish_alloc_permit.cta_group::2.sync.aligned;" ::: "memory");
  }
  asm volatile("tcgen05.fence::before_thread_sync;" ::: "memory");
  __syncthreads();
  cluster_sync_all();
  asm volatile("tcgen05.fence::after_thread_sync;" ::: "memory");
  const uint32_t tmem_base = *tmem_slot;

  if (warp == 0) {
    if (lane == 0) {
      asm volatile("prefetch.tensormap [%0];" ::"l"(reinterpret_cast<uint64_t>(&mapA)) : "memory");
      asm volatile("prefetch.tensormap [%0];" ::"l"(reinterpret_cast<uint64_t>(&mapB)) : "memory");
      uint32_t it = 0;
      long long w_empty = 0;
      const long long tstart = a.dbg ? clock64() : 0;
      for (long long t = pair; t < a.num_tiles; t += npairs) {
        if (a.tile_on && !a.tile_on[t]) continue;
        long long r = t;
        const int n_tile = (int)(r % a.nt); r /= a.nt;
        const int m_tile = (int)(r % a.mt); r /= a.mt;
        const int y = (int)(r % a.Y);
        const int z = (int)(r / a.Y);
        const int bnj = min(a.bn, a.n_mma - n_tile * a.bn);
        const int m0 = m_tile * 256 + (int)rank * TC_BM, n0 = n_tile * a.bn + (int)rank * (bnj >> 1);
        for (int kb = 0; kb < a.nkb; ++kb, ++it) {
          const int s = it % a.stages;
          const uint32_t use = it / a.stages;
          if (use > 0) {
            const long long c0 = a.dbg ? clock64() : 0;
            mbar_wait(&empty[s], (use - 1) & 1);
            if (a.dbg) w_empty += clock64() - c0;
          }
          uint8_t* sp = sStage + s * stage_bytes;
          const int tap = kb / a.kpt, ka = (kb - tap * a.kpt) * 2 * TC_BK;
          const int px = m0 + a.tap_dx[tap], ln = y + a.a_y0 + a.tap_dy[tap], pl = z + a.a_z0 + a.tap_dz[tap];
          const uint32_t lbar = smem_u32(&full[s]) & 0xFEFFFFFFu;
          if (rank == 0) mbar_expect_tx(&full[s], (uint32_t)(2 * stage_bytes));
          tma_load_4d_2sm(&mapA, lbar, sp, ka, px, a.a_swap ? pl : ln, a.a_swap ? ln : pl);
          tma_load_4d_2sm(&mapA, lbar, sp + TC_A_HALF, ka + TC_BK, px, a.a_swap ? pl : ln, a.a_swap ? ln : pl);
          tma_load_2d_2sm(&mapB, lbar, sp + 2 * TC_A_HALF, kb * 2 * TC_BK, n0);
          tma_load_2d_2sm(&mapB, lbar, sp + 2 * TC_A_HALF + b_half, kb * 2 * TC_BK + TC_BK, n0);
        }
      }
      if (a.dbg && rank == 0) { a.dbg[pair * 8 + 0] = (unsigned long long)w_empty; a.dbg[pair * 8 + 1] = (unsigned long long)(clock64() - tstart); }
    }
    __syncwarp();
  } else if (warp == 1) {
    if (rank == 0) {
      const uint32_t leader = elect_one();
      const uint32_t idesc0 = (1u << 4) | (1u << 7) | (1u << 10) | ((uint32_t)(256 >> 4) << 24);
      const uint32_t sStage_u = smem_u32(sStage);
      uint32_t it = 0, ti = 0;
      long long w_full = 0, w_tempty = 0;
      const long long tstart = a.dbg ? clock64() : 0;
      for (long long t = pair; t < a.num_tiles; t += npairs) {
        if (a.tile_on && !a.tile_on[t]) continue;
        const uint32_t b = ti & 1, buse = ti >> 1;
        const int bnj = min(a.bn, a.n_mma - (int)(t % a.nt) * a.bn);
        const uint32_t idesc = idesc0 | ((uint32_t)(bnj >> 3) << 17);
        long long c0 = a.dbg ? clock64() : 0;
        mbar_wait(&tempty[b], (buse & 1) ^ 1);
        if (a.dbg) w_tempty += clock64() - c0;
        asm volatile("tcgen05.fence::after_thread_sync;" ::: "memory");
        const uint32_t acc = tmem_base + b * 256;
        for (int kb = 0; kb < a.nkb; ++kb, ++it) {
          const int s = it % a.stages;
          c0 = a.dbg ? clock64() : 0;
          mbar_wait(&full[s], (it / a.stages) & 1);
          if (a.dbg) w_full += clock64() - c0;
          asm volatile("tcgen05.fence::after_thread_sync;" ::: "memory");
          const uint32_t sp = sStage_u + s * stage_bytes;
          const uint64_t ah = umma_desc(sp), al = umma_desc(sp + TC_A_HALF);
          const uint64_t wh = umma_desc(sp + 2 * TC_A_HALF), wl = umma_desc(sp + 2 * TC_A_HALF + b_half);
          const int nj = kb == a.nkb - 1 ? a.last_ksteps : 4;
#pragma unroll
          for (int j = 0; j < 4; ++j) {
            const uint64_t o = (uint64_t)(j * 2);
            const uint32_t on = (leader && j < nj) ? 1u : 0u;
            umma_bf16_2sm_elect(acc, al + o, wh + o, idesc, (kb | j) != 0, on);
            umma_bf16_2sm_elect(acc, ah + o, wl + o, idesc, 1, on);
            umma_bf16_2sm_elect(acc, ah + o, wh + o, idesc, 1, on);
          }
          if (leader) umma_commit_2sm(&empty[s]);
          __syncwarp();
        }
        if (leader) umma_commit_2sm(&tfull[b]);
        __syncwarp();
        ++ti;
      }
      if (a.dbg && leader) {
        a.dbg[pair * 8 + 2] = (unsigned long long)w_full; a.dbg[pair * 8 + 3] = (unsigned long long)w_tempty;
        a.dbg[pair * 8 + 4] = (unsigned long long)(clock64() - tstart);
      }
    }
  } else {
    const int q = warp & 3;
    const int G = nepi >> 2, grp = (warp - 2) >> 2;
    const int epi_threads = nepi * 32;
    uint32_t ti = 0;
    long long w_tfull = 0;
    for (int i = threadIdx.x - 64; i < a.nt * a.bn; i += epi_threads) {
      const int j = i / a.bn, c = i - j * a.bn, nn = i;
      const bool ok = nn < a.npad;
      float* cbw = s_const + j * 3 * a.bn;
      cbw[c] = ok ? __ldg(a.bias + nn) : 0.f;
      cbw[a.bn + c] = ok ? __ldg(a.alpha + nn) : 1.f;
      cbw[2 * a.bn + c] = (a.scale && ok) ? __ldg(a.scale + nn) : 1.f;
    }
    asm volatile("bar.sync 1, %0;" ::"r"(epi_threads) : "memory");
    const long long tstart = a.dbg ? clock64() : 0;
    for (long long t = pair; t < a.num_tiles; t += npairs) {
      if (a.tile_on && !a.tile_on[t]) continue;
      long long r = t;
      const int n_tile = (int)(r % a.nt); r /= a.nt;
      const int m_tile = (int)(r % a.mt); r /= a.mt;
      const int y = (int)(r % a.Y);
      const int z = (int)(r / a.Y);
      const int m0 = m_tile * 256 + (int)rank * TC_BM, n0 = n_tile * a.bn;
      const uint32_t b = ti & 1, buse = ti >> 1;
      const float* cb = s_const + n_tile * 3 * a.bn;
      const long long c0w = a.dbg ? clock64() : 0;
      mbar_wait(&tfull[b], buse & 1);
      if (a.dbg) w_tfull += clock64() - c0w;
      asm volatile("tcgen05.fence::after_thread_sync;" ::: "memory");
      float* ctile = a.C + (long long)z * a.c_zs + (long long)y * a.c_ys;
      const int mw = m0 + q * 32;
      uint8_t* stg = s_stage + (warp - 2) * 2560;
      uint8_t* mine = stg + lane * 80;
      uint32_t rr[3][16];
#pragma unroll
      for (int i = 0; i < 3; ++i) {
        const int c0 = grp * 16 + i * 16 * G;
        if (c0 < a.bn) tmem_ld16(rr[i], tmem_base + b * 256 + ((uint32_t)(q * 32) << 16) + (uint32_t)c0);
      }
      asm volatile("tcgen05.wait::ld.sync.aligned;" ::: "memory");
      asm volatile("tcgen05.fence::before_thread_sync;" ::: "memory");
      __syncwarp();
      if (lane == 0) mbar_arrive_cta(&tempty[b], 0);
      float* myrow = nullptr;
      if (a.out_split && mw + lane < a.M) {
        myrow = ctile + (long long)(mw + lane) * a.ldc;
        if (a.rowmap) {
          const int cr = __ldg(a.rowmap + ((long long)z * a.c_zs + (long long)y * a.c_ys + (long long)(mw + lane) * a.ldc));
          myrow = cr < 0 ? nullptr : a.C + (long long)cr * a.crow_ld;
        }
      }
#pragma unroll
      for (int i = 0; i < 3; ++i) {
        const int c0 = grp * 16 + i * 16 * G;
        if (c0 >= a.bn || n0 + c0 >= a.n_store) continue;
        if (n0 + c0 >= a.n_mma) {
#pragma unroll
          for (int kk = 0; kk < 16; ++kk) rr[i][kk] = 0u;
        }
        float v[16];
#pragma unroll
        for (int k4 = 0; k4 < 4; ++k4) {
          const float4 bi = *reinterpret_cast<const float4*>(cb + c0 + 4 * k4);
          const float4 al = *reinterpret_cast<const float4*>(cb + a.bn + c0 + 4 * k4);
          if (a.scale) {
            const float4 sc_ = *reinterpret_cast<const float4*>(cb + 2 * a.bn + c0 + 4 * k4);
            v[4 * k4 + 0] = prelu(fmaf(__uint_as_float(rr[i][4 * k4 + 0]), sc_.x, bi.x), al.x);
            v[4 * k4 + 1] = prelu(fmaf(__uint_as_float(rr[i][4 * k4 + 1]), sc_.y, bi.y), al.y);
            v[4 * k4 + 2] = prelu(fmaf(__uint_as_float(rr[i][4 * k4 + 2]), sc_.z, bi.z), al.z);
            v[4 * k4 + 3] = prelu(fmaf(__uint_as_float(rr[i][4 * k4 + 3]), sc_.w, bi.w), al.w);
          } else {
            v[4 * k4 + 0] = prelu(__uint_as_float(rr[i][4 * k4 + 0]) + bi.x, al.x);
            v[4 * k4 + 1] = prelu(__uint_as_float(rr[i][4 * k4 + 1]) + bi.y, al.y);
            v[4 * k4 + 2] = prelu(__uint_as_float(rr[i][4 * k4 + 2]) + bi.z, al.z);
            v[4 * k4 + 3] = prelu(__uint_as_float(rr[i][4 * k4 + 3]) + bi.w, al.w);
          }
        }
        const int ncol = a.c_col0 + n0 + c0;
        if (a.atlas && (ncol == 528 || ncol == 544)) {
          long long mrow = (long long)mw + lane;
          float at[15];
          if (mrow < a.M) {
            if (a.rowvox) mrow = __ldg(a.rowvox + mrow);
            const long long plane = (long long)a.ageo.by * a.ageo.bz;
            const int ix = (int)(mrow / plane);
            const int rem = (int)(mrow - (long long)ix * plane);
            const int iy = rem / a.ageo.bz, iz = rem - iy * a.ageo.bz;
            const long long vx = ((long long)(a.ageo.x0 + ix) * a.ageo.Y + (a.ageo.y0 + iy)) * a.ageo.Z + (a.ageo.z0 + iz);
#pragma unroll
            for (int c = 0; c < 15; ++c) at[c] = __ldg(a.atlas + vx * 15 + c);
            float sum = __fadd_rn(__fadd_rn(__fadd_rn(at[0], at[1]), __fadd_rn(at[2], at[3])),
                                  __fadd_rn(__fadd_rn(at[4], at[5]), __fadd_rn(at[6], at[7])));
#pragma unroll
            for (int k = 8; k < 15; ++k) sum = __fadd_rn(sum, at[k]);
            if (sum == 0.f) at[14] = 1.f;
          } else {
#pragma unroll
            for (int c = 0; c < 15; ++c) at[c] = 0.f;
          }
          if (ncol == 528) { v[12] = at[0]; v[13] = at[1]; v[14] = at[2]; v[15] = at[3]; }
          else {
#pragma unroll
            for (int k = 0; k < 16; ++k) v[k] = k < 11 ? at[4 + k] : 0.f;
          }
        }
        if (a.out_split) {
          uint32_t hi[8], lo[8];
#pragma unroll
          for (int k = 0; k < 8; ++k) split2(v[2 * k], v[2 * k + 1], hi[k], lo[k]);
          *reinterpret_cast<uint4*>(mine) = make_uint4(hi[0], hi[1], hi[2], hi[3]);
          *reinterpret_cast<uint4*>(mine + 16) = make_uint4(hi[4], hi[5], hi[6], hi[7]);
          *reinterpret_cast<uint4*>(mine + 32) = make_uint4(lo[0], lo[1], lo[2], lo[3]);
          *reinterpret_cast<uint4*>(mine + 48) = make_uint4(lo[4], lo[5], lo[6], lo[7]);
          __syncwarp();
          const int boff = (ncol >> 6) * 128 + (ncol & 63);
#pragma unroll
          for (int j = 0; j < 4; ++j) {
            const int half = j >> 1, row = (j & 1) * 16 + (lane >> 1), part = lane & 1;
            const uint4 d = *reinterpret_cast<const uint4*>(stg + row * 80 + half * 32 + part * 16);
            float* crow = reinterpret_cast<float*>(__shfl_sync(0xffffffffu, reinterpret_cast<unsigned long long>(myrow), row));
            if (crow) *reinterpret_cast<uint4*>(reinterpret_cast<__nv_bfloat16*>(crow) + boff + half * 64 + part * 8) = d;
          }
        } else {
#pragma unroll
          for (int k = 0; k < 4; ++k)
            *reinterpret_cast<float4*>(mine + 16 * k) = make_float4(v[4 * k], v[4 * k + 1], v[4 * k + 2], v[4 * k + 3]);
          __syncwarp();
#pragma unroll
          for (int j = 0; j < 4; ++j) {
            const int row = j * 8 + (lane >> 2), part = lane & 3;
            const float4 d = *reinterpret_cast<const float4*>(stg + row * 80 + part * 16);
            if (mw + row < a.M) *reinterpret_cast<float4*>(ctile + (long long)(mw + row) * a.ldc + ncol + part * 4) = d;
          }
        }
        __syncwarp();
      }
      ++ti;
    }
    if (a.dbg && rank == 0 && threadIdx.x == 64) {
      a.dbg[pair * 8 + 5] = (unsigned long long)w_tfull; a.dbg[pair * 8 + 6] = (unsigned long long)(clock64() - tstart);
      a.dbg[pair * 8 + 7] = ti;
    }
  }
  asm volatile("tcgen05.fence::before_thread_sync;" ::: "memory");
  __syncthreads();
  cluster_sync_all();
  if (warp == 1) {
    asm volatile("tcgen05.fence::after_thread_sync;" ::: "memory");
    asm volatile("tcgen05.dealloc.cta_group::2.sync.aligned.b32 %0, %1;" ::"r"(tmem_base), "r"(512) : "memory");
  }
}

__global__ void split_rows_kernel(const float* __restrict__ in, int64_t rows, float* __restrict__ out) {
  const int64_t i = (int64_t)blockIdx.x * blockDim.x + threadIdx.x;
  if (i >= rows * (kFeatLd / 4)) return;
  const int64_t m = i / (kFeatLd / 4);
  const int n = (int)(i - m * (kFeatLd / 4)) * 4;
  const float4 v = __ldg(reinterpret_cast<const float4*>(in + m * kFeatLd + n));
  store_split4(out + m * kFeatLd, n, v.x, v.y, v.z, v.w);
}
int launch_split_rows(sc_ctx* ctx, const float* in, int64_t rows, float* out, cudaStream_t st) {
  const int64_t work = rows * (kFeatLd / 4);
  split_rows_kernel<<<(unsigned)((work + 255) / 256), 256, 0, st>>>(in, rows, out);
  ctx->launches++;
  SC_CUDA(cudaGetLastError());
  return SC_OK;
}

__global__ void tile_flags_kernel(const int* __restrict__ rowmap, long long num_tiles, int nt, int mt, int Y, int M, long long ldc,
                                  long long c_ys, long long c_zs, unsigned char* __restrict__ flags) {
  const long long t = (long long)blockIdx.x * (blockDim.x >> 5) + (threadIdx.x >> 5);
  if (t >= num_tiles) return;
  long long r = t / nt;
  const int m_tile = (int)(r % mt); r /= mt;
  const int y = (int)(r % Y);
  const int z = (int)(r / Y);
  const int lane = threadIdx.x & 31;
  bool any = false;
  for (int k = lane; k < 256; k += 32) {
    const int m = m_tile * 256 + k;
    if (m < M && __ldg(rowmap + ((long long)z * c_zs + (long long)y * c_ys + (long long)m * ldc)) >= 0) any = true;
  }
  any = __any_sync(0xffffffffu, any);
  if (lane == 0) flags[t] = any ? 1 : 0;
}

int tc_init(sc_ctx* ctx) {
  void* fn = nullptr;
  cudaDriverEntryPointQueryResult q;
  cudaError_t e = cudaGetDriverEntryPoint("cuTensorMapEncodeTiled", &fn, cudaEnableDefault, &q);
  if (e != cudaSuccess || q != cudaDriverEntryPointSuccess || !fn) {
    cudaGetLastError();
    set_error("tcgen05 back-end: cuTensorMapEncodeTiled unavailable");
    return SC_ERR_UNSUPPORTED;
  }
  TcState* s = new TcState();
  s->encode = reinterpret_cast<EncodeTiledFn>(fn);
  ctx->tc_state = s;
  return SC_OK;
}

void tc_destroy(sc_ctx* ctx) {
  delete reinterpret_cast<TcState*>(ctx->tc_state);
  ctx->tc_state = nullptr;
}

static int pick_bn(int n_store) {
  int best = 16, best_cost = 1 << 30;
  for (int bn = 192; bn >= 32; bn -= 16) {
    const int tiles = (n_store + bn - 1) / bn;
    const int cost = tiles * bn * 4 + tiles * 128;
    if (cost < best_cost) { best_cost = cost; best = bn; }
  }
  return best;
}

int launch_gemm_tc(sc_ctx* ctx, const GemmProblem& p, const GemmW& w, cudaStream_t st) {
  TcState* s = reinterpret_cast<TcState*>(ctx->tc_state);
  SC_CHECK(s != nullptr, SC_ERR_UNSUPPORTED, "tcgen05 back-end not initialised");
  if (p.M <= 0 || p.Y <= 0 || p.Z <= 0) return SC_OK;
  SC_CHECK(p.kc % TC_BK == 0 && p.ntaps * p.kc == w.Kpad && p.n_store % 4 == 0 && p.n_store <= w.Npad, SC_ERR_ARG,
           "gemm_tc: bad geometry kc=%d ntaps=%d Kpad=%d n_store=%d", p.kc, p.ntaps, w.Kpad, p.n_store);
  TcArgs a;
  a.kpt = p.kc / TC_BK;
  a.c_col0 = p.c_col0;
  a.nkb = p.ntaps * a.kpt;
  a.bn = pick_bn(p.n_store);
  a.sm_on = 0;
  a.atlas = p.atlas; a.ageo = p.ageo;
  a.rowmap = p.rowmap; a.rowvox = p.rowvox; a.crow_ld = 0; a.tile_on = nullptr;
  if (p.sm) {
    SC_CHECK(p.n_store == 16 && p.ntaps == 1, SC_ERR_ARG, "gemm_tc: the softmax epilogue needs a 16-column layer");
    a.bn = 16; a.sm_on = 1; a.sm = *p.sm;
  }
  a.nt = (p.n_store + a.bn - 1) / a.bn;
  a.mt = (p.M + TC_BM - 1) / TC_BM;
  a.Y = p.Y; a.M = p.M; a.npad = w.Npad;
  a.n_store = (p.n_store + 15) & ~15;
  if (p.atlas) a.n_store = 576;
  SC_CHECK(p.c_col0 % 16 == 0, SC_ERR_ARG, "gemm_tc: c_col0 must be a multiple of 16");
  a.a_y0 = p.a_y0; a.a_z0 = p.a_z0; a.a_swap = p.a_swap;
  for (int t = 0; t < 9; ++t) { a.tap_dx[t] = t < p.ntaps ? p.tap_dx[t] : 0; a.tap_dy[t] = t < p.ntaps ? p.tap_dy[t] : 0; a.tap_dz[t] = t < p.ntaps ? p.tap_dz[t] : 0; }
  a.C = p.C; a.ldc = p.ldc; a.c_ys = p.c_ys; a.c_zs = p.c_zs;
  if (p.rowmap) {
    SC_CHECK(p.out_split && p.ldc % kFeatLd == 0 && p.c_ys % kFeatLd == 0 && p.c_zs % kFeatLd == 0, SC_ERR_ARG, "gemm_tc: rowmap needs split rows of kFeatLd floats");
    a.crow_ld = kFeatLd; a.ldc = p.ldc / kFeatLd; a.c_ys = p.c_ys / kFeatLd; a.c_zs = p.c_zs / kFeatLd;
  }
  a.bias = w.bias; a.alpha = w.alpha; a.scale = w.scale; a.out_split = p.out_split;
  const bool pair = a.bn >= 128 && a.bn % 16 == 0 && !p.sm;
  SC_CHECK(!p.rowmap || pair, SC_ERR_ARG, "gemm_tc: the row map is implemented in the CTA-pair kernel");
  SC_CHECK(!p.atlas || (pair && p.c_col0 == 0 && p.n_store == 540 && w.Npad == 576), SC_ERR_ARG, "gemm_tc: the atlas epilogue is for FC1 in the CTA-pair kernel");
  const long long blocks = (long long)a.mt * a.nt * p.Y * p.Z;
  SC_CHECK(blocks < (1ll << 31), SC_ERR_ARG, "gemm_tc: grid too large");
  a.num_tiles = blocks;
  a.dbg = (ctx->tc_timing_cls == p.prof_cls) ? ctx->tc_timing_buf : nullptr;
  a.last_ksteps = 4;
  if (p.ntaps == 1 && w.k_used > w.Kpad - TC_BK && w.k_used <= w.Kpad) a.last_ksteps = (w.k_used - (w.Kpad - TC_BK) + 15) / 16;
  int stage_bytes;
  size_t smem = 0;
  if (pair) {
    a.mt = (p.M + 255) / 256;
    a.num_tiles = (long long)a.mt * a.nt * p.Y * p.Z;
    a.epi_warps = 16;
    stage_bytes = 2 * TC_A_HALF + 2 * (a.bn / 2) * 128;
    SC_CHECK(a.nt <= 4, SC_ERR_ARG, "gemm_tc: more than 4 n-tiles in the CTA-pair kernel");
    const int cst = (a.nt > 2 ? a.nt : 2) * 3 * a.bn * 4;
    const int budget = 227 * 1024 - 1024 - 192 - 16 - cst - a.epi_warps * 2560;
    a.stages = budget / stage_bytes;
    if (a.stages > 6) a.stages = 6;
    SC_CHECK(a.stages >= 2, SC_ERR_ARG, "gemm_tc: pair tile too wide");
    smem = 1024 + (size_t)a.stages * stage_bytes + (2 * a.stages + 4) * 8 + 32 + cst + (size_t)a.epi_warps * 2560;
  } else {
    a.epi_warps = a.bn > 64 ? 16 : 8;
    const int budget = 227 * 1024 - 1024 - 128 - 16 - 2 * 3 * a.bn * 4 - a.epi_warps * 2560;
    stage_bytes = 2 * TC_A_HALF + 2 * a.bn * 128;
    a.stages = budget / stage_bytes;
    if (a.stages > 6) a.stages = 6;
    SC_CHECK(a.stages >= 2, SC_ERR_ARG, "gemm_tc: tile too wide for two stages (bn=%d)", a.bn);
    smem = 1024 + (size_t)a.stages * stage_bytes + (2 * a.stages + 4) * 8 + 16 + 2 * 3 * a.bn * 4 + (size_t)a.epi_warps * 2560;
  }

  CUtensorMap mapA, mapB;
  {
    cuuint64_t dims[4] = {(cuuint64_t)p.a_dims[0] * 2, (cuuint64_t)p.a_dims[1], (cuuint64_t)p.a_dims[2], (cuuint64_t)p.a_dims[3]};
    cuuint64_t strides[3] = {(cuuint64_t)p.a_strides[0] * 4, (cuuint64_t)p.a_strides[1] * 4, (cuuint64_t)p.a_strides[2] * 4};
    cuuint32_t box[4] = {TC_BK, TC_BM, 1, 1};
    cuuint32_t es[4] = {1, 1, 1, 1};
    CUresult r = s->encode(&mapA, CU_TENSOR_MAP_DATA_TYPE_BFLOAT16, 4, const_cast<float*>(p.a_base), dims, strides, box, es,
                           CU_TENSOR_MAP_INTERLEAVE_NONE, CU_TENSOR_MAP_SWIZZLE_128B, CU_TENSOR_MAP_L2_PROMOTION_L2_256B,
                           CU_TENSOR_MAP_FLOAT_OOB_FILL_NONE);
    SC_CHECK(r == CUDA_SUCCESS, SC_ERR_CUDA, "gemm_tc: cuTensorMapEncodeTiled(A) failed with %d (dims %llu %llu %llu %llu)", (int)r,
             (unsigned long long)dims[0], (unsigned long long)dims[1], (unsigned long long)dims[2], (unsigned long long)dims[3]);
  }
  {
    cuuint64_t dims[2] = {(cuuint64_t)w.Kpad * 2, (cuuint64_t)w.Npad};
    cuuint64_t strides[1] = {(cuuint64_t)w.Kpad * 4};
    cuuint32_t box[2] = {TC_BK, (cuuint32_t)(pair ? a.bn / 2 : a.bn)};
    cuuint32_t es[2] = {1, 1};
    CUresult r = s->encode(&mapB, CU_TENSOR_MAP_DATA_TYPE_BFLOAT16, 2, w.w_nk, dims, strides, box, es,
                           CU_TENSOR_MAP_INTERLEAVE_NONE, CU_TENSOR_MAP_SWIZZLE_128B, CU_TENSOR_MAP_L2_PROMOTION_L2_256B,
                           CU_TENSOR_MAP_FLOAT_OOB_FILL_NONE);
    SC_CHECK(r == CUDA_SUCCESS, SC_ERR_CUDA, "gemm_tc: cuTensorMapEncodeTiled(B) failed with %d", (int)r);
  }
  SC_TRY(ensure_smem_attr(ctx, reinterpret_cast<const void*>(gemm_tc_persistent_kernel), 227 * 1024));
  SC_TRY(ensure_smem_attr(ctx, reinterpret_cast<const void*>(gemm_tc_pair_kernel), 227 * 1024));
  SC_CHECK(smem <= 227 * 1024, SC_ERR_ARG, "gemm_tc: shared memory budget exceeded (%zu)", smem);
  ProfScope prof(ctx, p.prof_cls, st);
  a.n_mma = a.nt * a.bn;
  if (pair && p.ntaps == 1) {
    int real = (w.N + 15) & ~15;
    if (real > p.n_store) real = (p.n_store + 15) & ~15;
    if (real - (a.nt - 1) * a.bn >= 32 && real <= a.nt * a.bn) a.n_mma = real;
  }
  if (pair && p.rowmap) {
    if (ctx->tile_flags_cap < (size_t)a.num_tiles) {
      if (ctx->tile_flags) cudaFree(ctx->tile_flags);
      ctx->tile_flags = nullptr; ctx->tile_flags_cap = 0;
      const size_t cap = ((size_t)a.num_tiles + 65535) & ~(size_t)65535;
      SC_CUDA(cudaMalloc(&ctx->tile_flags, cap));
      ctx->tile_flags_cap = cap;
    }
    tile_flags_kernel<<<(unsigned)((a.num_tiles + 7) / 8), 256, 0, st>>>(p.rowmap, a.num_tiles, a.nt, a.mt, a.Y, a.M, a.ldc, a.c_ys, a.c_zs, ctx->tile_flags);
    ctx->launches++;
    a.tile_on = ctx->tile_flags;
  }
  if (pair) {
    long long pairs = a.num_tiles < ctx->sm_count / 2 ? a.num_tiles : ctx->sm_count / 2;
    gemm_tc_pair_kernel<<<(unsigned)(2 * pairs), 64 + 32 * a.epi_warps, smem, st>>>(mapA, mapB, a);
  } else {
    const unsigned grid = (unsigned)(blocks < ctx->sm_count ? blocks : ctx->sm_count);
    gemm_tc_persistent_kernel<<<grid, 64 + 32 * a.epi_warps, smem, st>>>(mapA, mapB, a);
  }
  ctx->launches++;
  SC_CUDA(cudaGetLastError());
  return SC_OK;
}

}
```

sub-cortical_segmentation_b200/csrc/patch_forward.cu:

```cuda
#include "common.cuh"

namespace sc {

struct PatchW {
  const float* c1_w;
  const float* w[5];
  const float* scale[5];
  const float* shift[5];
  const float* alpha[5];
};

constexpr int C1_LD = 32;
constexpr int S_IN = 0;
constexpr int S_C1 = 1024;
constexpr int S_P1 = S_C1 + 19200;
constexpr int S_P2 = S_P1 + 4480;
constexpr int S_TOTAL = S_P2 + 1000;
constexpr size_t PATCH_SMEM = S_TOTAL * sizeof(float);

__global__ void __launch_bounds__(256) branch_patch_kernel(const float* __restrict__ patches, const PatchW W,
                                                           float* __restrict__ c5_out, int round_out) {
  extern __shared__ __align__(16) float sm[];
  float* s_in = sm + S_IN;
  float* s_c1 = sm + S_C1;
  float* s_c3 = sm + S_C1;
  float* s_p1 = sm + S_P1;
  float* s_p2 = sm + S_P2;
  const int tid = threadIdx.x;
  const int64_t n = blockIdx.x;
  reinterpret_cast<float4*>(s_in)[tid] = __ldg(reinterpret_cast<const float4*>(patches + n * 1024) + tid);
  __syncthreads();

  for (int idx = tid; idx < 900; idx += 256) {
    const int py = idx / 30, px = idx - py * 30;
    float x[9];
#pragma unroll
    for (int ky = 0; ky < 3; ++ky)
#pragma unroll
      for (int kx = 0; kx < 3; ++kx) x[ky * 3 + kx] = s_in[(py + ky) * 32 + px + kx];
#pragma unroll 5
    for (int co = 0; co < 20; ++co) {
      float a = 0.f;
#pragma unroll
      for (int t = 0; t < 9; ++t) a = fmaf(x[t], __ldg(W.c1_w + t * 20 + co), a);
      s_c1[(co * 30 + py) * C1_LD + px] = prelu(fmaf(a, __ldg(W.scale[0] + co), __ldg(W.shift[0] + co)), __ldg(W.alpha[0] + co));
    }
  }
  __syncthreads();

  for (int item = tid; item < 5 * 196; item += 256) {
    const int cgp = item / 196, pp = item - cgp * 196, ppy = pp / 14, ppx = pp - ppy * 14;
    float acc[4][4];
#pragma unroll
    for (int p = 0; p < 4; ++p)
#pragma unroll
      for (int c = 0; c < 4; ++c) acc[p][c] = 0.f;
#pragma unroll 2
    for (int ci = 0; ci < 20; ++ci) {
      float x[4][4];
#pragma unroll
      for (int r = 0; r < 4; ++r) {
        const float2* src = reinterpret_cast<const float2*>(s_c1 + (ci * 30 + 2 * ppy + r) * C1_LD + 2 * ppx);
        const float2 a = src[0], b = src[1];
        x[r][0] = a.x; x[r][1] = a.y; x[r][2] = b.x; x[r][3] = b.y;
      }
#pragma unroll
      for (int ky = 0; ky < 3; ++ky)
#pragma unroll
        for (int kx = 0; kx < 3; ++kx) {
          const float4 w = __ldg(reinterpret_cast<const float4*>(W.w[1] + (ci * 9 + ky * 3 + kx) * 20 + cgp * 4));
          const float wv[4] = {w.x, w.y, w.z, w.w};
#pragma unroll
          for (int dy = 0; dy < 2; ++dy)
#pragma unroll
            for (int dx = 0; dx < 2; ++dx)
#pragma unroll
              for (int c = 0; c < 4; ++c) acc[dy * 2 + dx][c] = fmaf(x[dy + ky][dx + kx], wv[c], acc[dy * 2 + dx][c]);
        }
    }
#pragma unroll
    for (int c = 0; c < 4; ++c) {
      const int co = cgp * 4 + c;
      const float s = __ldg(W.scale[1] + co), h = __ldg(W.shift[1] + co), al = __ldg(W.alpha[1] + co);
      float m = prelu(fmaf(acc[0][c], s, h), al);
#pragma unroll
      for (int p = 1; p < 4; ++p) m = fmaxf(m, prelu(fmaf(acc[p][c], s, h), al));
      s_p1[(co * 14 + ppy) * 16 + ppx] = m;
    }
  }
  __syncthreads();

  if (tid < 5 * 36) {
    const int cgp = tid / 36, seg = tid - cgp * 36, row = seg / 3, c0 = (seg - row * 3) * 4;
    float acc[4][8];
#pragma unroll
    for (int p = 0; p < 4; ++p)
#pragma unroll
      for (int c = 0; c < 8; ++c) acc[p][c] = 0.f;
#pragma unroll 1
    for (int ci = 0; ci < 20; ++ci) {
#pragma unroll
      for (int ky = 0; ky < 3; ++ky) {
        const float* src = s_p1 + (ci * 14 + row + ky) * 16 + c0;
        const float4 a = *reinterpret_cast<const float4*>(src);
        const float2 b = *reinterpret_cast<const float2*>(src + 4);
        const float x[6] = {a.x, a.y, a.z, a.w, b.x, b.y};
#pragma unroll
        for (int kx = 0; kx < 3; ++kx) {
          const float4* wp = reinterpret_cast<const float4*>(W.w[2] + (ci * 9 + ky * 3 + kx) * 40 + cgp * 8);
          const float4 w0 = __ldg(wp), w1 = __ldg(wp + 1);
          const float wv[8] = {w0.x, w0.y, w0.z, w0.w, w1.x, w1.y, w1.z, w1.w};
#pragma unroll
          for (int p = 0; p < 4; ++p)
#pragma unroll
            for (int c = 0; c < 8; ++c) acc[p][c] = fmaf(x[p + kx], wv[c], acc[p][c]);
        }
      }
    }
#pragma unroll
    for (int c = 0; c < 8; ++c) {
      const int co = cgp * 8 + c;
      const float s = __ldg(W.scale[2] + co), h = __ldg(W.shift[2] + co), al = __ldg(W.alpha[2] + co);
#pragma unroll
      for (int p = 0; p < 4; ++p) s_c3[(co * 12 + row) * 12 + c0 + p] = prelu(fmaf(acc[p][c], s, h), al);
    }
  }
  __syncthreads();

  if (tid < 250) {
    const int cgp = tid / 25, pp = tid - cgp * 25, ppy = pp / 5, ppx = pp - ppy * 5;
    float acc[4][4];
#pragma unroll
    for (int p = 0; p < 4; ++p)
#pragma unroll
      for (int c = 0; c < 4; ++c) acc[p][c] = 0.f;
#pragma unroll 2
    for (int ci = 0; ci < 40; ++ci) {
      float x[4][4];
#pragma unroll
      for (int r = 0; r < 4; ++r) {
        const float2* src = reinterpret_cast<const float2*>(s_c3 + (ci * 12 + 2 * ppy + r) * 12 + 2 * ppx);
        const float2 a = src[0], b = src[1];
        x[r][0] = a.x; x[r][1] = a.y; x[r][2] = b.x; x[r][3] = b.y;
      }
#pragma unroll
      for (int ky = 0; ky < 3; ++ky)
#pragma unroll
        for (int kx = 0; kx < 3; ++kx) {
          const float4 w = __ldg(reinterpret_cast<const float4*>(W.w[3] + (ci * 9 + ky * 3 + kx) * 40 + cgp * 4));
          const float wv[4] = {w.x, w.y, w.z, w.w};
#pragma unroll
          for (int dy = 0; dy < 2; ++dy)
#pragma unroll
            for (int dx = 0; dx < 2; ++dx)
#pragma unroll
              for (int c = 0; c < 4; ++c) acc[dy * 2 + dx][c] = fmaf(x[dy + ky][dx + kx], wv[c], acc[dy * 2 + dx][c]);
        }
    }
#pragma unroll
    for (int c = 0; c < 4; ++c) {
      const int co = cgp * 4 + c;
      const float s = __ldg(W.scale[3] + co), h = __ldg(W.shift[3] + co), al = __ldg(W.alpha[3] + co);
      float m = prelu(fmaf(acc[0][c], s, h), al);
#pragma unroll
      for (int p = 1; p < 4; ++p) m = fmaxf(m, prelu(fmaf(acc[p][c], s, h), al));
      s_p2[co * 25 + pp] = m;
    }
  }
  __syncthreads();

  float* out = c5_out + n * kFeatLd;
  if (tid < 135) {
    const int cgp = tid / 9, px = tid - cgp * 9, py = px / 3, pxx = px - py * 3;
    float acc[4] = {0.f, 0.f, 0.f, 0.f};
#pragma unroll 4
    for (int ci = 0; ci < 40; ++ci) {
#pragma unroll
      for (int ky = 0; ky < 3; ++ky)
#pragma unroll
        for (int kx = 0; kx < 3; ++kx) {
          const float x = s_p2[ci * 25 + (py + ky) * 5 + pxx + kx];
          const float4 w = __ldg(reinterpret_cast<const float4*>(W.w[4] + (ci * 9 + ky * 3 + kx) * 60 + cgp * 4));
          acc[0] = fmaf(x, w.x, acc[0]); acc[1] = fmaf(x, w.y, acc[1]);
          acc[2] = fmaf(x, w.z, acc[2]); acc[3] = fmaf(x, w.w, acc[3]);
        }
    }
#pragma unroll
    for (int c = 0; c < 4; ++c) {
      const int co = cgp * 4 + c;
      const float v = prelu(fmaf(acc[c], __ldg(W.scale[4] + co), __ldg(W.shift[4] + co)), __ldg(W.alpha[4] + co));
      store_row1(out, co * 9 + px, round_out, v);
    }
  } else if (tid >= 220) {
    store_row1(out, 540 + (tid - 220), round_out, 0.f);
  }
}

int launch_branch_patches(sc_ctx* ctx, int b, const float* patches, int64_t n, float* c5_out, cudaStream_t st) {
  if (n == 0) return SC_OK;
  SC_TRY(ensure_smem_attr(ctx, reinterpret_cast<const void*>(branch_patch_kernel), (int)PATCH_SMEM));
  PatchW W;
  W.c1_w = ctx->br[b].c1_w;
  for (int l = 0; l < 5; ++l) {
    W.w[l] = ctx->br[b].conv_w[l];
    W.scale[l] = ctx->br[b].scale[l]; W.shift[l] = ctx->br[b].shift[l]; W.alpha[l] = ctx->br[b].alpha[l];
  }
  SC_CHECK(n < (1ll << 31), SC_ERR_ARG, "forward: batch too large");
  ProfScope prof(ctx, PC_PATCH_BRANCH, st);
  branch_patch_kernel<<<(unsigned)n, 256, PATCH_SMEM, st>>>(patches, W, c5_out, ctx->gemm_backend == 1);
  ctx->launches++;
  SC_CUDA(cudaGetLastError());
  return SC_OK;
}

__global__ void atlas_rows_kernel(const float* __restrict__ in4, int64_t n, float* __restrict__ h1, int split) {
  const int64_t i = (int64_t)blockIdx.x * blockDim.x + threadIdx.x;
  if (i >= n * 9) return;
  const int64_t m = i / 9;
  const int q = (int)(i - m * 9);
  float a[4] = {0.f, 0.f, 0.f, 0.f};
#pragma unroll
  for (int k = 0; k < 4; ++k)
    if (q * 4 + k < 15) a[k] = __ldg(in4 + m * 15 + q * 4 + k);
  store_row4(h1 + m * kH1Ld, 540 + 4 * q, split, a[0], a[1], a[2], a[3]);
}

int forward_patches(sc_ctx* ctx, const float* in1, const float* in2, const float* in3, const float* in4, int64_t n,
                    float* proba, int32_t* label, cudaStream_t st) {
  const bool tc = ctx->gemm_backend == 1;
  const int64_t chunk = 32768, sub = 4096;
  const size_t row_floats = 3 * kFeatLd + kFeatLd + kH1Ld + kH2Ld;
  const int64_t cmax = n < chunk ? n : chunk;
  const size_t head_bytes = (size_t)cmax * row_floats * sizeof(float) + 1024;
  const size_t conv_bytes = tc ? branch_patches_tc_bytes(cmax < sub ? cmax : sub) : 0;
  SC_TRY(ensure_ws(ctx->ws, head_bytes + conv_bytes));
  float* c5 = reinterpret_cast<float*>(ctx->ws.ptr);
  float* feats = c5 + (size_t)cmax * 3 * kFeatLd;
  float* h1 = feats + (size_t)cmax * kFeatLd;
  float* h2 = h1 + (size_t)cmax * kH1Ld;
  float* conv_scratch = reinterpret_cast<float*>(reinterpret_cast<char*>(ctx->ws.ptr) + ((head_bytes + 255) & ~(size_t)255));
  const float* ins[3] = {in1, in2, in3};
  for (int64_t s = 0; s < n; s += chunk) {
    const int64_t m = n - s < chunk ? n - s : chunk;
    for (int b = 0; b < 3; ++b) {
      if (tc) {
        for (int64_t t = 0; t < m; t += sub) {
          const int64_t mm = m - t < sub ? m - t : sub;
          SC_TRY(branch_patches_tc(ctx, b, ins[b] + (s + t) * 1024, mm, conv_scratch, feats + t * kFeatLd, st));
        }
        continue;
      }
      float* c5b = c5 + (size_t)b * cmax * kFeatLd;
      SC_TRY(launch_branch_patches(ctx, b, ins[b] + s * 1024, m, c5b, st));
      GemmProblem p;
      gemm_problem_rows(p, c5b, kFeatLd, kFeatLd, (int)m);
      p.C = feats; p.ldc = kFeatLd; p.c_col0 = b * 192;
      p.n_store = 192; p.out_split = 0; p.prof_cls = PC_GEMM_D1;
      SC_TRY(launch_gemm(ctx, p, ctx->br[b].d1, st));
    }
    GemmProblem p;
    gemm_problem_rows(p, feats, kFeatLd, kFeatLd, (int)m);
    p.C = h1; p.ldc = kH1Ld; p.n_store = 540; p.out_split = tc ? 1 : 0;
    p.prof_cls = PC_GEMM_FC1;
    SC_TRY(tc ? launch_gemm_tc(ctx, p, ctx->fc1, st) : launch_gemm(ctx, p, ctx->fc1, st));
    { ProfScope prof(ctx, PC_ATLAS, st);
      atlas_rows_kernel<<<(unsigned)((m * 9 + 255) / 256), 256, 0, st>>>(in4 + s * 15, m, h1, tc ? 1 : 0); }
    ctx->launches++;
    SC_CUDA(cudaGetLastError());
    gemm_problem_rows(p, h1, kH1Ld, kH1Ld, (int)m);
    p.C = h2; p.ldc = kH2Ld; p.n_store = kH2Ld; p.out_split = 0;
    p.prof_cls = PC_GEMM_FC2;
    SC_TRY(tc ? launch_gemm_tc(ctx, p, ctx->fc2, st) : launch_gemm(ctx, p, ctx->fc2, st));
    SC_TRY(launch_out_softmax(ctx, h2, m, proba ? proba + s * 15 : nullptr, label ? label + s : nullptr, nullptr,
                              nullptr, nullptr, st));
  }
  return SC_OK;
}

}
```

sub-cortical_segmentation_b200/csrc/weights.cu:

```cuda
#include <math.h>
#include <string.h>

#include "common.cuh"

namespace sc {

static uint16_t bf16_rn(float x) {
  uint32_t u;
  memcpy(&u, &x, 4);
  if ((u & 0x7f800000u) == 0x7f800000u) return (uint16_t)(u >> 16);
  u += 0x7fffu + ((u >> 16) & 1u);
  return (uint16_t)(u >> 16);
}
static float bf16_to_float(uint16_t h) {
  uint32_t u = (uint32_t)h << 16;
  float r;
  memcpy(&r, &u, 4);
  return r;
}

struct Arena {
  std::vector<float> host;
  size_t alloc(size_t n) {
    size_t o = host.size();
    n = (n + 63) & ~(size_t)63;
    host.resize(o + n, 0.f);
    return o;
  }
};

struct GemmOff { size_t kn, nk, bias, alpha, scale; };

static GemmOff make_gemm(Arena& A, GemmW& g, int K, int N, int Kpad, int Npad) {
  g.K = K; g.N = N; g.Kpad = Kpad; g.Npad = Npad;
  GemmOff o;
  o.kn = A.alloc((size_t)Kpad * Npad);
  o.nk = A.alloc((size_t)Npad * Kpad);
  o.bias = A.alloc(Npad);
  o.alpha = A.alloc(Npad);
  o.scale = A.alloc(Npad);
  for (int n = 0; n < Npad; ++n) { A.host[o.scale + n] = 1.f; A.host[o.alpha + n] = 1.f; }
  return o;
}
static void set_w(Arena& A, const GemmOff& o, const GemmW& g, int k, int n, float v) {
  A.host[o.kn + (size_t)k * g.Npad + n] = v;
  uint16_t* row = reinterpret_cast<uint16_t*>(&A.host[o.nk + (size_t)n * g.Kpad]);
  const uint16_t hi = bf16_rn(v);
  row[(k >> 6) * 128 + (k & 63)] = hi;
  row[(k >> 6) * 128 + 64 + (k & 63)] = bf16_rn(v - bf16_to_float(hi));
}
static void bind(GemmW& g, const GemmOff& o, float* base) {
  g.w_kn = base + o.kn; g.w_nk = base + o.nk; g.bias = base + o.bias; g.alpha = base + o.alpha; g.scale = base + o.scale;
}

int derive_weights(sc_ctx* ctx, cudaStream_t st) {
  const ParamOff& P = ctx->off;
  std::vector<float> h(P.total);
  SC_CUDA(cudaMemcpyAsync(h.data(), ctx->params, sizeof(float) * P.total, cudaMemcpyDeviceToHost, st));
  SC_CUDA(cudaStreamSynchronize(st));

  Arena A;
  struct BOff { size_t c1, conv[5], scale[5], shift[5], alpha[5], sw[5], swp[5]; GemmOff d1, d1d; } bo[3];
  GemmOff fc1o, fc2o, outo;
  size_t outw, outb;
  for (int b = 0; b < 3; ++b) {
    const BranchOff& B = P.br[b];
    bo[b].c1 = A.alloc(9 * 20);
    for (int t = 0; t < 9; ++t)
      for (int co = 0; co < 20; ++co) A.host[bo[b].c1 + t * 20 + co] = ctx->br[b].c1_host.w[t * 20 + co] = h[B.convW[0] + co * 9 + (8 - t)];
    for (int l = 0; l < 5; ++l) {
      const int ci_n = kConvCin[l], co_n = kConvCout[l];
      if (l > 0) {
        bo[b].conv[l] = A.alloc((size_t)ci_n * 9 * co_n);
        for (int co = 0; co < co_n; ++co)
          for (int ci = 0; ci < ci_n; ++ci)
            for (int t = 0; t < 9; ++t)
              A.host[bo[b].conv[l] + ((size_t)ci * 9 + t) * co_n + co] = h[B.convW[l] + ((size_t)co * ci_n + ci) * 9 + (8 - t)];
      }
      bo[b].scale[l] = A.alloc(64);
      bo[b].shift[l] = A.alloc(64);
      bo[b].alpha[l] = A.alloc(64);
      if (l > 0) {
        SweepW& S = ctx->br[b].conv_sw[l];
        S.ksteps = (ci_n + 15) / 16; S.bn = (co_n + 15) & ~15; S.npanels = (9 * S.ksteps + 3) / 4;
        bo[b].sw[l] = A.alloc((size_t)S.npanels * 2 * S.bn * 32);
        bo[b].swp[l] = A.alloc((size_t)S.npanels * 2 * S.bn * 32);
        uint16_t* pw = reinterpret_cast<uint16_t*>(&A.host[bo[b].sw[l]]);
        uint16_t* pp = reinterpret_cast<uint16_t*>(&A.host[bo[b].swp[l]]);
        const int hb = S.bn / 2;
        for (int co = 0; co < co_n; ++co)
          for (int ci = 0; ci < ci_n; ++ci)
            for (int t = 0; t < 9; ++t) {
              const float v = h[B.convW[l] + ((size_t)co * ci_n + ci) * 9 + (8 - t)];
              const int gk = t * S.ksteps + ci / 16, kk = (gk & 3) * 16 + (ci & 15);
              const uint16_t hi = bf16_rn(v);
              pw[((size_t)(gk >> 2) * 2 * S.bn + co) * 64 + kk] = hi;
              pw[((size_t)(gk >> 2) * 2 * S.bn + S.bn + co) * 64 + kk] = bf16_rn(v - bf16_to_float(hi));
              const size_t prow = ((size_t)(gk >> 2) * 2 + co / hb) * S.bn + co % hb;
              pp[prow * 64 + kk] = hi;
              pp[(prow + hb) * 64 + kk] = bf16_rn(v - bf16_to_float(hi));
            }
      }
      for (int c = 0; c < co_n; ++c) {
        const float beta = h[B.bn[l][0] + c], gamma = h[B.bn[l][1] + c], mean = h[B.bn[l][2] + c], inv = h[B.bn[l][3] + c];
        const float s = gamma * inv;
        A.host[bo[b].scale[l] + c] = s;
        A.host[bo[b].shift[l] + c] = beta - mean * s;
        A.host[bo[b].alpha[l] + c] = h[B.alpha[l] + c];
        if (l == 0) { ctx->br[b].c1_host.scale[c] = s; ctx->br[b].c1_host.shift[c] = beta - mean * s; ctx->br[b].c1_host.alpha[c] = h[B.alpha[l] + c]; }
      }
    }
    bo[b].d1 = make_gemm(A, ctx->br[b].d1, 540, 180, kFeatLd, 192);
    bo[b].d1d = make_gemm(A, ctx->br[b].d1_dense, kD1K, 180, kD1K, 192);
    for (int k = 0; k < 540; ++k)
      for (int n = 0; n < 180; ++n) {
        const float v = h[B.d1W + (size_t)k * 180 + n];
        set_w(A, bo[b].d1, ctx->br[b].d1, k, n, v);
        const int c = k / 9, t = k % 9;
        set_w(A, bo[b].d1d, ctx->br[b].d1_dense, t * kC5Ld + c, n, v);
      }
    for (int n = 0; n < 192; ++n) {
      const float bias = n < 180 ? h[B.d1b + n] : 0.f, al = n < 180 ? h[B.d1alpha + n] : 1.f;
      A.host[bo[b].d1.bias + n] = A.host[bo[b].d1d.bias + n] = bias;
      A.host[bo[b].d1.alpha + n] = A.host[bo[b].d1d.alpha + n] = al;
    }
  }
  fc1o = make_gemm(A, ctx->fc1, 540, 540, kFeatLd, 576);
  for (int k = 0; k < 540; ++k)
    for (int n = 0; n < 540; ++n) set_w(A, fc1o, ctx->fc1, (k / 180) * 192 + (k % 180), n, h[P.fc1W + (size_t)k * 540 + n]);
  for (int n = 0; n < 576; ++n) {
    A.host[fc1o.bias + n] = n < 540 ? h[P.fc1b + n] : 0.f;
    A.host[fc1o.alpha + n] = n < 540 ? h[P.a1 + n] : 1.f;
  }
  fc2o = make_gemm(A, ctx->fc2, 555, 270, kH1Ld, kH2Ld);
  ctx->fc2.k_used = 555;
  for (int b = 0; b < 3; ++b) ctx->br[b].d1.k_used = 540;
  ctx->fc1.k_used = 0;
  for (int k = 0; k < 555; ++k)
    for (int n = 0; n < 270; ++n) set_w(A, fc2o, ctx->fc2, k, n, h[P.fc2W + (size_t)k * 270 + n]);
  for (int n = 0; n < kH2Ld; ++n) {
    A.host[fc2o.bias + n] = n < 270 ? h[P.fc2b + n] : 0.f;
    A.host[fc2o.alpha + n] = n < 270 ? h[P.a2 + n] : 1.f;
  }
  outo = make_gemm(A, ctx->outl, 270, 15, kH2LdTc, 16);
  for (int k = 0; k < 270; ++k)
    for (int n = 0; n < 15; ++n) set_w(A, outo, ctx->outl, k, n, h[P.outW + k * 15 + n]);
  for (int n = 0; n < 15; ++n) A.host[outo.bias + n] = h[P.outb + n];
  outw = A.alloc(270 * 16);
  outb = A.alloc(16);
  for (int k = 0; k < 270; ++k)
    for (int n = 0; n < 15; ++n) A.host[outw + k * 16 + n] = h[P.outW + k * 15 + n];
  for (int n = 0; n < 15; ++n) A.host[outb + n] = h[P.outb + n];

  if (ctx->derived_floats < A.host.size()) {
    if (ctx->derived) cudaFree(ctx->derived);
    ctx->derived = nullptr;
    SC_CUDA(cudaMalloc(&ctx->derived, A.host.size() * sizeof(float)));
    ctx->derived_floats = A.host.size();
  }
  SC_CUDA(cudaMemcpyAsync(ctx->derived, A.host.data(), A.host.size() * sizeof(float), cudaMemcpyHostToDevice, st));
  SC_CUDA(cudaStreamSynchronize(st));
  float* base = ctx->derived;
  for (int b = 0; b < 3; ++b) {
    ctx->br[b].c1_w = base + bo[b].c1;
    for (int l = 0; l < 5; ++l) {
      ctx->br[b].conv_w[l] = l > 0 ? base + bo[b].conv[l] : nullptr;
      ctx->br[b].scale[l] = base + bo[b].scale[l];
      ctx->br[b].shift[l] = base + bo[b].shift[l];
      ctx->br[b].alpha[l] = base + bo[b].alpha[l];
    }
    for (int l = 1; l < 5; ++l) {
      SweepW& S = ctx->br[b].conv_sw[l];
      S.panels = base + bo[b].sw[l]; S.panels_pair = base + bo[b].swp[l]; S.scale = ctx->br[b].scale[l]; S.shift = ctx->br[b].shift[l]; S.alpha = ctx->br[b].alpha[l];
    }
    bind(ctx->br[b].d1, bo[b].d1, base);
    bind(ctx->br[b].d1_dense, bo[b].d1d, base);
  }
  bind(ctx->fc1, fc1o, base);
  bind(ctx->fc2, fc2o, base);
  bind(ctx->outl, outo, base);
  ctx->out_w = base + outw;
  ctx->out_b = base + outb;
  return SC_OK;
}

}
```

Before: 151.1 million.

## Fuse out_layer and softmax into the FC2 tensor-core GEMM epilogue

The separate h2 buffer write, its memset, and the second tensor-core GEMM for the 15-class output layer are removed. The FC2 CTA-pair kernel gains a templated epilogue that applies PReLU to each accumulator tile, multiplies by out-layer weights held in shared memory, and keeps 15 logits per row. It walks all N-tiles of a row block within one unit, reduces partial sums across epilogue groups through shared memory, then runs softmax and stores the result. This removes a large intermediate round trip through global memory and one kernel launch per slab. In exchange the epilogue does FP32 FMA work on CUDA cores and adds extra barriers, and it schedules only one unit per row block, which means fewer parallel units.

```diff
diff --git a/sub-cortical_segmentation_b200/csrc/common.cuh b/sub-cortical_segmentation_b200/csrc/common.cuh
--- a/sub-cortical_segmentation_b200/csrc/common.cuh
+++ b/sub-cortical_segmentation_b200/csrc/common.cuh
@@ -80,7 +80,6 @@
 constexpr int kH1Ld = 576;
 constexpr int kH2 = 270;
 constexpr int kH2Ld = 272;
-constexpr int kH2LdTc = 320;
 constexpr int kC5Ld = 64;
 constexpr int kD1K = 9 * kC5Ld;
 
@@ -148,7 +147,6 @@
   size_t derived_floats = 0;
   sc::BranchW br[3];
   sc::GemmW fc1, fc2;
-  sc::GemmW outl;
   float* out_w = nullptr;
   float* out_b = nullptr;
   sc::Workspace ws;
@@ -376,6 +374,28 @@
                int64_t n, float* out2, cudaStream_t st);
 
 __device__ __forceinline__ float prelu(float x, float a) { return x > 0.f ? x : a * x; }
+__device__ __forceinline__ void softmax_store(float (&z)[15], long long o, float* proba, int32_t* label32, uint8_t* label8) {
+  float mx = z[0];
+#pragma unroll
+  for (int c = 1; c < 15; ++c) mx = fmaxf(mx, z[c]);
+  float sum = 0.f;
+#pragma unroll
+  for (int c = 0; c < 15; ++c) { z[c] = expf(z[c] - mx); sum += z[c]; }
+  const float inv = 1.f / sum;
+  int best = 0;
+  float bp = z[0] * inv;
+#pragma unroll
+  for (int c = 0; c < 15; ++c) {
+    z[c] *= inv;
+    if (z[c] > bp) { bp = z[c]; best = c; }
+  }
+  if (proba) {
+#pragma unroll
+    for (int c = 0; c < 15; ++c) proba[o * 15 + c] = z[c];
+  }
+  if (label32) label32[o] = best;
+  if (label8) label8[o] = (uint8_t)best;
+}
 __device__ __forceinline__ void store_split4(float* row, int n, float v0, float v1, float v2, float v3) {
   __nv_bfloat16* r = reinterpret_cast<__nv_bfloat16*>(row) + (n >> 6) * 128 + (n & 63);
   const __nv_bfloat16 h0 = __float2bfloat16_rn(v0), h1 = __float2bfloat16_rn(v1), h2 = __float2bfloat16_rn(v2), h3 = __float2bfloat16_rn(v3);
diff --git a/sub-cortical_segmentation_b200/csrc/dense.cu b/sub-cortical_segmentation_b200/csrc/dense.cu
--- a/sub-cortical_segmentation_b200/csrc/dense.cu
+++ b/sub-cortical_segmentation_b200/csrc/dense.cu
@@ -328,8 +328,7 @@
   const size_t rows_max = (size_t)slab * plane;
   const size_t feat_bytes = align256(rows_max * kFeatLd * sizeof(float));
   const size_t h1_bytes = align256(rows_max * kH1Ld * sizeof(float));
-  const int h2ld = tc ? kH2LdTc : kH2Ld;
-  const size_t h2_bytes = align256(rows_max * h2ld * sizeof(float));
+  const size_t h2_bytes = tc ? 0 : align256(rows_max * kH2Ld * sizeof(float));
   const int nslabs = (bx + slab - 1) / slab;
   bool compact = tc && cand != nullptr && ctx->tc_compact && nslabs <= 4096;
   const size_t nbox = (size_t)bx * plane;
@@ -438,7 +437,6 @@
 
   int atlas_waited = 0;
   OutGeo og = {b[0], b[2], b[4], by, bz, Y, Z};
-  if (tc) SC_CUDA(cudaMemsetAsync(h2, 0, h2_bytes, st));
   for (int ix0 = 0; ix0 < bx; ix0 += slab) {
     const int nx = bx - ix0 < slab ? bx - ix0 : slab;
     const int64_t rows = (int64_t)nx * plane;
@@ -510,18 +508,16 @@
     }
     SC_CUDA(cudaGetLastError());
     gemm_problem_rows(p, h1, kH1Ld, kH1Ld, (int)rows_fc);
-    p.C = h2; p.ldc = h2ld; p.n_store = kH2Ld; p.out_split = tc ? 1 : 0;
     p.prof_cls = PC_GEMM_FC2;
-    SC_TRY(tc ? launch_gemm_tc(ctx, p, ctx->fc2, st) : launch_gemm(ctx, p, ctx->fc2, st));
     OutGeo og2 = og;
     og2.x0 = b[0] + ix0;
     if (tc) {
       SoftmaxOut smo = {proba_vol, nullptr, label_vol, cand, og2, 1, compact ? rowvox + slab_base : nullptr};
-      gemm_problem_rows(p, h2, h2ld, h2ld, (int)rows_fc);
-      p.C = nullptr; p.ldc = 0; p.n_store = 16; p.out_split = 0; p.sm = &smo;
-      p.prof_cls = PC_OUT;
-      SC_TRY(launch_gemm_tc(ctx, p, ctx->outl, st));
+      p.C = nullptr; p.ldc = 0; p.n_store = kH2Ld; p.sm = &smo;
+      SC_TRY(launch_gemm_tc(ctx, p, ctx->fc2, st));
     } else {
+      p.C = h2; p.ldc = kH2Ld; p.n_store = kH2Ld;
+      SC_TRY(launch_gemm(ctx, p, ctx->fc2, st));
       SC_TRY(launch_out_softmax(ctx, h2, rows, proba_vol, nullptr, label_vol, cand, &og2, st));
     }
   }
diff --git a/sub-cortical_segmentation_b200/csrc/gemm_simt.cu b/sub-cortical_segmentation_b200/csrc/gemm_simt.cu
--- a/sub-cortical_segmentation_b200/csrc/gemm_simt.cu
+++ b/sub-cortical_segmentation_b200/csrc/gemm_simt.cu
@@ -142,26 +142,7 @@
       }
     }
   }
-  float mx = z[0];
-#pragma unroll
-  for (int c = 1; c < 15; ++c) mx = fmaxf(mx, z[c]);
-  float sum = 0.f;
-#pragma unroll
-  for (int c = 0; c < 15; ++c) { z[c] = expf(z[c] - mx); sum += z[c]; }
-  const float inv = 1.f / sum;
-  int best = 0;
-  float bp = z[0] * inv;
-#pragma unroll
-  for (int c = 0; c < 15; ++c) {
-    z[c] *= inv;
-    if (z[c] > bp) { bp = z[c]; best = c; }
-  }
-  if (proba) {
-#pragma unroll
-    for (int c = 0; c < 15; ++c) proba[o * 15 + c] = z[c];
-  }
-  if (label) label[o] = best;
-  if (label8) label8[o] = (uint8_t)best;
+  softmax_store(z, o, proba, label, label8);
 }
 
 int launch_out_softmax(sc_ctx* ctx, const float* h2, int64_t n, float* proba, int32_t* label, uint8_t* label8,
diff --git a/sub-cortical_segmentation_b200/csrc/gemm_tc.cu b/sub-cortical_segmentation_b200/csrc/gemm_tc.cu
--- a/sub-cortical_segmentation_b200/csrc/gemm_tc.cu
+++ b/sub-cortical_segmentation_b200/csrc/gemm_tc.cu
@@ -43,9 +43,14 @@
   const unsigned char* tile_on;
   const float* atlas;
   OutGeo ageo;
-  int sm_on;
   SoftmaxOut sm;
+  const float* out_w;
+  const float* out_b;
 };
+
+constexpr int kOutWFloats = kH2Ld * 16;
+constexpr int kOutPartFloats = 3 * 15 * TC_BM;
+static_assert((kOutWFloats + 16 + kOutPartFloats) * 4 <= 16 * 2560, "fused out_layer scratch exceeds the store-transpose area");
 
 
 __global__ void __launch_bounds__(576, 1)
@@ -190,59 +195,6 @@
       const int mw = m0 + q * 32;
       uint8_t* stg = s_stage + (warp - 2) * 2560;
       uint8_t* mine = stg + lane * 80;
-      if (a.sm_on) {
-        if (grp == 0) {
-          uint32_t rr[16];
-          const uint32_t taddr = tmem_base + b * 256 + ((uint32_t)(q * 32) << 16);
-          asm volatile(
-              "tcgen05.ld.sync.aligned.32x32b.x16.b32 {%0, %1, %2, %3, %4, %5, %6, %7, %8, %9, %10, %11, %12, %13, %14, %15}, [%16];"
-              : "=r"(rr[0]), "=r"(rr[1]), "=r"(rr[2]), "=r"(rr[3]), "=r"(rr[4]), "=r"(rr[5]), "=r"(rr[6]), "=r"(rr[7]), "=r"(rr[8]),
-                "=r"(rr[9]), "=r"(rr[10]), "=r"(rr[11]), "=r"(rr[12]), "=r"(rr[13]), "=r"(rr[14]), "=r"(rr[15])
-              : "r"(taddr));
-          asm volatile("tcgen05.wait::ld.sync.aligned;" ::: "memory");
-          long long m = (long long)mw + lane;
-          bool ok = m < a.M;
-          if (ok && a.sm.rowvox) m = __ldg(a.sm.rowvox + m);
-          long long o = m;
-          if (ok && a.sm.use_geo) {
-            const long long plane = (long long)a.sm.geo.by * a.sm.geo.bz;
-            const int ix = (int)(m / plane);
-            const int rem = (int)(m - (long long)ix * plane);
-            const int iy = rem / a.sm.geo.bz, iz = rem - iy * a.sm.geo.bz;
-            o = ((long long)(a.sm.geo.x0 + ix) * a.sm.geo.Y + (a.sm.geo.y0 + iy)) * a.sm.geo.Z + (a.sm.geo.z0 + iz);
-            if (a.sm.mask && a.sm.mask[o] == 0) ok = false;
-          }
-          if (ok) {
-            float zz[15];
-#pragma unroll
-            for (int c = 0; c < 15; ++c) zz[c] = __uint_as_float(rr[c]) + cb[c];
-            float mx = zz[0];
-#pragma unroll
-            for (int c = 1; c < 15; ++c) mx = fmaxf(mx, zz[c]);
-            float sum = 0.f;
-#pragma unroll
-            for (int c = 0; c < 15; ++c) { zz[c] = expf(zz[c] - mx); sum += zz[c]; }
-            const float inv = 1.f / sum;
-            int best = 0;
-            float bp = zz[0] * inv;
-#pragma unroll
-            for (int c = 0; c < 15; ++c) {
-              zz[c] *= inv;
-              if (zz[c] > bp) { bp = zz[c]; best = c; }
-            }
-            if (a.sm.proba) {
-#pragma unroll
-              for (int c = 0; c < 15; ++c) a.sm.proba[o * 15 + c] = zz[c];
-            }
-            if (a.sm.label32) a.sm.label32[o] = best;
-            if (a.sm.label8) a.sm.label8[o] = (uint8_t)best;
-          }
-        }
-        asm volatile("tcgen05.fence::before_thread_sync;" ::: "memory");
-        __syncwarp();
-        if (lane == 0) mbar_arrive(&tempty[b]);
-        continue;
-      }
       for (int c0 = grp * 16; c0 < a.bn; c0 += 16 * G) {
         uint32_t rr[16];
         const uint32_t taddr = tmem_base + b * 256 + ((uint32_t)(q * 32) << 16) + (uint32_t)c0;
@@ -315,6 +267,7 @@
   }
 }
 
+template <bool FUSED_OUT>
 __global__ void __cluster_dims__(2, 1, 1) __launch_bounds__(576, 1)
 gemm_tc_pair_kernel(const __grid_constant__ CUtensorMap mapA, const __grid_constant__ CUtensorMap mapB, const TcArgs a) {
   extern __shared__ uint8_t smem_raw[];
@@ -335,7 +288,9 @@
   const int warp = threadIdx.x >> 5, lane = threadIdx.x & 31;
   const uint32_t rank = cluster_ctarank();
   const int nepi = (blockDim.x >> 5) - 2;
-  const long long pair = (long long)(blockIdx.x >> 1), npairs = (long long)(gridDim.x >> 1);
+  const int pair = (int)(blockIdx.x >> 1), npairs = (int)(gridDim.x >> 1);
+  const int per = FUSED_OUT ? a.nt : 1;
+  const int units = (int)(a.num_tiles / per);
 
   if (threadIdx.x == 0) {
     for (int s = 0; s < a.stages; ++s) { mbar_init(&full[s], 1); mbar_init(&empty[s], 1); }
@@ -359,7 +314,9 @@
       uint32_t it = 0;
       long long w_empty = 0;
       const long long tstart = a.dbg ? clock64() : 0;
-      for (long long t = pair; t < a.num_tiles; t += npairs) {
+      for (int u = pair; u < units; u += npairs)
+      for (int jt = 0; jt < per; ++jt) {
+        const int t = u * per + jt;
         if (a.tile_on && !a.tile_on[t]) continue;
         long long r = t;
         const int n_tile = (int)(r % a.nt); r /= a.nt;
@@ -398,7 +355,9 @@
       uint32_t it = 0, ti = 0;
       long long w_full = 0, w_tempty = 0;
       const long long tstart = a.dbg ? clock64() : 0;
-      for (long long t = pair; t < a.num_tiles; t += npairs) {
+      for (int u = pair; u < units; u += npairs)
+      for (int jt = 0; jt < per; ++jt) {
+        const int t = u * per + jt;
         if (a.tile_on && !a.tile_on[t]) continue;
         const uint32_t b = ti & 1, buse = ti >> 1;
         const int bnj = min(a.bn, a.n_mma - (int)(t % a.nt) * a.bn);
@@ -452,9 +411,19 @@
       cbw[a.bn + c] = ok ? __ldg(a.alpha + nn) : 1.f;
       cbw[2 * a.bn + c] = (a.scale && ok) ? __ldg(a.scale + nn) : 1.f;
     }
+    float* s_ow = reinterpret_cast<float*>(s_stage);
+    float* s_ob = s_ow + kOutWFloats;
+    float* s_part = s_ob + 16;
+    if (FUSED_OUT) {
+      for (int i = threadIdx.x - 64; i < kOutWFloats + 16; i += epi_threads)
+        s_ow[i] = i < 270 * 16 ? __ldg(a.out_w + i) : (i >= kOutWFloats ? __ldg(a.out_b + i - kOutWFloats) : 0.f);
+    }
     asm volatile("bar.sync 1, %0;" ::"r"(epi_threads) : "memory");
+    float logit[15];
     const long long tstart = a.dbg ? clock64() : 0;
-    for (long long t = pair; t < a.num_tiles; t += npairs) {
+    for (int u = pair; u < units; u += npairs)
+    for (int jt = 0; jt < per; ++jt) {
+      const int t = u * per + jt;
       if (a.tile_on && !a.tile_on[t]) continue;
       long long r = t;
       const int n_tile = (int)(r % a.nt); r /= a.nt;
@@ -472,6 +441,71 @@
       const int mw = m0 + q * 32;
       uint8_t* stg = s_stage + (warp - 2) * 2560;
       uint8_t* mine = stg + lane * 80;
+      if (FUSED_OUT) {
+        if (jt == 0) {
+#pragma unroll
+          for (int c = 0; c < 15; ++c) logit[c] = 0.f;
+        }
+#pragma unroll
+        for (int i = 0; i < 3; ++i) {
+          const int c0 = grp * 16 + i * 16 * G;
+          if (c0 >= a.bn || n0 + c0 >= a.n_store) continue;
+          uint32_t r[16];
+          tmem_ld16(r, tmem_base + b * 256 + ((uint32_t)(q * 32) << 16) + (uint32_t)c0);
+          asm volatile("tcgen05.wait::ld.sync.aligned;" ::: "memory");
+          const float4* w4 = reinterpret_cast<const float4*>(s_ow + (n0 + c0) * 16);
+#pragma unroll
+          for (int k = 0; k < 16; ++k) {
+            const float x = prelu(fmaf(__uint_as_float(r[k]), cb[2 * a.bn + c0 + k], cb[c0 + k]), cb[a.bn + c0 + k]);
+            const float4 w0 = w4[4 * k], w1 = w4[4 * k + 1], w2 = w4[4 * k + 2], w3 = w4[4 * k + 3];
+            logit[0] = fmaf(x, w0.x, logit[0]); logit[1] = fmaf(x, w0.y, logit[1]);
+            logit[2] = fmaf(x, w0.z, logit[2]); logit[3] = fmaf(x, w0.w, logit[3]);
+            logit[4] = fmaf(x, w1.x, logit[4]); logit[5] = fmaf(x, w1.y, logit[5]);
+            logit[6] = fmaf(x, w1.z, logit[6]); logit[7] = fmaf(x, w1.w, logit[7]);
+            logit[8] = fmaf(x, w2.x, logit[8]); logit[9] = fmaf(x, w2.y, logit[9]);
+            logit[10] = fmaf(x, w2.z, logit[10]); logit[11] = fmaf(x, w2.w, logit[11]);
+            logit[12] = fmaf(x, w3.x, logit[12]); logit[13] = fmaf(x, w3.y, logit[13]);
+            logit[14] = fmaf(x, w3.z, logit[14]);
+          }
+        }
+        asm volatile("tcgen05.fence::before_thread_sync;" ::: "memory");
+        __syncwarp();
+        if (lane == 0) mbar_arrive_cta(&tempty[b], 0);
+        ++ti;
+        if (jt == per - 1) {
+          const int crow = q * 32 + lane;
+          if (grp > 0) {
+#pragma unroll
+            for (int c = 0; c < 15; ++c) s_part[((grp - 1) * 15 + c) * TC_BM + crow] = logit[c];
+          }
+          asm volatile("bar.sync 1, %0;" ::"r"(epi_threads) : "memory");
+          if (grp == 0) {
+#pragma unroll
+            for (int g = 0; g < 3; ++g)
+#pragma unroll
+              for (int c = 0; c < 15; ++c) logit[c] += s_part[(g * 15 + c) * TC_BM + crow];
+          }
+          asm volatile("bar.sync 1, %0;" ::"r"(epi_threads) : "memory");
+          long long m = (long long)mw + lane;
+          bool ok = grp == 0 && m < a.M;
+          if (ok && a.sm.rowvox) m = __ldg(a.sm.rowvox + m);
+          long long o = m;
+          if (ok && a.sm.use_geo) {
+            const long long plane = (long long)a.sm.geo.by * a.sm.geo.bz;
+            const int ix = (int)(m / plane);
+            const int rem = (int)(m - (long long)ix * plane);
+            const int iy = rem / a.sm.geo.bz, iz = rem - iy * a.sm.geo.bz;
+            o = ((long long)(a.sm.geo.x0 + ix) * a.sm.geo.Y + (a.sm.geo.y0 + iy)) * a.sm.geo.Z + (a.sm.geo.z0 + iz);
+            if (a.sm.mask && a.sm.mask[o] == 0) ok = false;
+          }
+          if (ok) {
+#pragma unroll
+            for (int c = 0; c < 15; ++c) logit[c] += s_ob[c];
+            softmax_store(logit, o, a.sm.proba, a.sm.label32, a.sm.label8);
+          }
+        }
+        continue;
+      }
       uint32_t rr[3][16];
 #pragma unroll
       for (int i = 0; i < 3; ++i) {
@@ -666,12 +700,13 @@
   a.c_col0 = p.c_col0;
   a.nkb = p.ntaps * a.kpt;
   a.bn = pick_bn(p.n_store);
-  a.sm_on = 0;
+  a.out_w = ctx->out_w; a.out_b = ctx->out_b;
   a.atlas = p.atlas; a.ageo = p.ageo;
   a.rowmap = p.rowmap; a.rowvox = p.rowvox; a.crow_ld = 0; a.tile_on = nullptr;
   if (p.sm) {
-    SC_CHECK(p.n_store == 16 && p.ntaps == 1, SC_ERR_ARG, "gemm_tc: the softmax epilogue needs a 16-column layer");
-    a.bn = 16; a.sm_on = 1; a.sm = *p.sm;
+    SC_CHECK(p.n_store == kH2Ld && p.ntaps == 1 && p.c_col0 == 0 && !p.out_split && !p.rowmap && !p.atlas && w.Npad == kH2Ld,
+             SC_ERR_ARG, "gemm_tc: the out_layer epilogue is for fc_2");
+    a.sm = *p.sm;
   }
   a.nt = (p.n_store + a.bn - 1) / a.bn;
   a.mt = (p.M + TC_BM - 1) / TC_BM;
@@ -687,8 +722,9 @@
     a.crow_ld = kFeatLd; a.ldc = p.ldc / kFeatLd; a.c_ys = p.c_ys / kFeatLd; a.c_zs = p.c_zs / kFeatLd;
   }
   a.bias = w.bias; a.alpha = w.alpha; a.scale = w.scale; a.out_split = p.out_split;
-  const bool pair = a.bn >= 128 && a.bn % 16 == 0 && !p.sm;
+  const bool pair = a.bn >= 128 && a.bn % 16 == 0;
   SC_CHECK(!p.rowmap || pair, SC_ERR_ARG, "gemm_tc: the row map is implemented in the CTA-pair kernel");
+  SC_CHECK(!p.sm || pair, SC_ERR_ARG, "gemm_tc: the out_layer epilogue is implemented in the CTA-pair kernel");
   SC_CHECK(!p.atlas || (pair && p.c_col0 == 0 && p.n_store == 540 && w.Npad == 576), SC_ERR_ARG, "gemm_tc: the atlas epilogue is for FC1 in the CTA-pair kernel");
   const long long blocks = (long long)a.mt * a.nt * p.Y * p.Z;
   SC_CHECK(blocks < (1ll << 31), SC_ERR_ARG, "gemm_tc: grid too large");
@@ -743,7 +779,8 @@
     SC_CHECK(r == CUDA_SUCCESS, SC_ERR_CUDA, "gemm_tc: cuTensorMapEncodeTiled(B) failed with %d", (int)r);
   }
   SC_TRY(ensure_smem_attr(ctx, reinterpret_cast<const void*>(gemm_tc_persistent_kernel), 227 * 1024));
-  SC_TRY(ensure_smem_attr(ctx, reinterpret_cast<const void*>(gemm_tc_pair_kernel), 227 * 1024));
+  SC_TRY(ensure_smem_attr(ctx, reinterpret_cast<const void*>(gemm_tc_pair_kernel<false>), 227 * 1024));
+  SC_TRY(ensure_smem_attr(ctx, reinterpret_cast<const void*>(gemm_tc_pair_kernel<true>), 227 * 1024));
   SC_CHECK(smem <= 227 * 1024, SC_ERR_ARG, "gemm_tc: shared memory budget exceeded (%zu)", smem);
   ProfScope prof(ctx, p.prof_cls, st);
   a.n_mma = a.nt * a.bn;
@@ -765,8 +802,10 @@
     a.tile_on = ctx->tile_flags;
   }
   if (pair) {
-    long long pairs = a.num_tiles < ctx->sm_count / 2 ? a.num_tiles : ctx->sm_count / 2;
-    gemm_tc_pair_kernel<<<(unsigned)(2 * pairs), 64 + 32 * a.epi_warps, smem, st>>>(mapA, mapB, a);
+    const long long units = p.sm ? a.num_tiles / a.nt : a.num_tiles;
+    const long long pairs = units < ctx->sm_count / 2 ? units : ctx->sm_count / 2;
+    if (p.sm) gemm_tc_pair_kernel<true><<<(unsigned)(2 * pairs), 64 + 32 * a.epi_warps, smem, st>>>(mapA, mapB, a);
+    else gemm_tc_pair_kernel<false><<<(unsigned)(2 * pairs), 64 + 32 * a.epi_warps, smem, st>>>(mapA, mapB, a);
   } else {
     const unsigned grid = (unsigned)(blocks < ctx->sm_count ? blocks : ctx->sm_count);
     gemm_tc_persistent_kernel<<<grid, 64 + 32 * a.epi_warps, smem, st>>>(mapA, mapB, a);
diff --git a/sub-cortical_segmentation_b200/csrc/patch_forward.cu b/sub-cortical_segmentation_b200/csrc/patch_forward.cu
--- a/sub-cortical_segmentation_b200/csrc/patch_forward.cu
+++ b/sub-cortical_segmentation_b200/csrc/patch_forward.cu
@@ -229,7 +229,7 @@
                     float* proba, int32_t* label, cudaStream_t st) {
   const bool tc = ctx->gemm_backend == 1;
   const int64_t chunk = 32768, sub = 4096;
-  const size_t row_floats = 3 * kFeatLd + kFeatLd + kH1Ld + kH2Ld;
+  const size_t row_floats = 3 * kFeatLd + kFeatLd + kH1Ld + (tc ? 0 : kH2Ld);
   const int64_t cmax = n < chunk ? n : chunk;
   const size_t head_bytes = (size_t)cmax * row_floats * sizeof(float) + 1024;
   const size_t conv_bytes = tc ? branch_patches_tc_bytes(cmax < sub ? cmax : sub) : 0;
@@ -268,9 +268,15 @@
     ctx->launches++;
     SC_CUDA(cudaGetLastError());
     gemm_problem_rows(p, h1, kH1Ld, kH1Ld, (int)m);
-    p.C = h2; p.ldc = kH2Ld; p.n_store = kH2Ld; p.out_split = 0;
-    p.prof_cls = PC_GEMM_FC2;
-    SC_TRY(tc ? launch_gemm_tc(ctx, p, ctx->fc2, st) : launch_gemm(ctx, p, ctx->fc2, st));
+    p.n_store = kH2Ld; p.prof_cls = PC_GEMM_FC2;
+    if (tc) {
+      SoftmaxOut smo = {proba ? proba + s * 15 : nullptr, label ? label + s : nullptr, nullptr, nullptr, OutGeo{}, 0, nullptr};
+      p.C = nullptr; p.ldc = 0; p.sm = &smo;
+      SC_TRY(launch_gemm_tc(ctx, p, ctx->fc2, st));
+      continue;
+    }
+    p.C = h2; p.ldc = kH2Ld;
+    SC_TRY(launch_gemm(ctx, p, ctx->fc2, st));
     SC_TRY(launch_out_softmax(ctx, h2, m, proba ? proba + s * 15 : nullptr, label ? label + s : nullptr, nullptr,
                               nullptr, nullptr, st));
   }
diff --git a/sub-cortical_segmentation_b200/csrc/weights.cu b/sub-cortical_segmentation_b200/csrc/weights.cu
--- a/sub-cortical_segmentation_b200/csrc/weights.cu
+++ b/sub-cortical_segmentation_b200/csrc/weights.cu
@@ -61,7 +61,7 @@
 
   Arena A;
   struct BOff { size_t c1, conv[5], scale[5], shift[5], alpha[5], sw[5], swp[5]; GemmOff d1, d1d; } bo[3];
-  GemmOff fc1o, fc2o, outo;
+  GemmOff fc1o, fc2o;
   size_t outw, outb;
   for (int b = 0; b < 3; ++b) {
     const BranchOff& B = P.br[b];
@@ -142,10 +142,6 @@
     A.host[fc2o.bias + n] = n < 270 ? h[P.fc2b + n] : 0.f;
     A.host[fc2o.alpha + n] = n < 270 ? h[P.a2 + n] : 1.f;
   }
-  outo = make_gemm(A, ctx->outl, 270, 15, kH2LdTc, 16);
-  for (int k = 0; k < 270; ++k)
-    for (int n = 0; n < 15; ++n) set_w(A, outo, ctx->outl, k, n, h[P.outW + k * 15 + n]);
-  for (int n = 0; n < 15; ++n) A.host[outo.bias + n] = h[P.outb + n];
   outw = A.alloc(270 * 16);
   outb = A.alloc(16);
   for (int k = 0; k < 270; ++k)
@@ -178,7 +174,6 @@
   }
   bind(ctx->fc1, fc1o, base);
   bind(ctx->fc2, fc2o, base);
-  bind(ctx->outl, outo, base);
   ctx->out_w = base + outw;
   ctx->out_b = base + outb;
   return SC_OK;
```

Measured after the change: 158.3 million, median of 6. 1.05x the previous value.
